# MarToonLi/StableDiffusionEO

Hardware: AMD Instinct MI355X
Metric: 512x512 canny2image images/sec (20 DDIM steps); ms per UNet step reported alongside (higher is better)
Workload: dtype f16; 1 GPU; SD1.5 + ControlNet-canny 512x512, batch=1 per GPU (CFG pair fused, N=2), 20 DDIM steps + VAE decode, fp16 storage / fp32 accumulate (BASELINE configs[1]); model_config=sd15, ddim_steps=20, parallelism=dp1 (image index -> rank, RCCL all_gather of final latents), weights=seeded synthetic (no checkpoint in the container)

## Files before the change

### stablediffusioneo_amd/csrc/api_ops.hip

```cpp
#include <stdarg.h>

#include "../../include/sdeo.h"
#include "sdeo_internal.h"
#include "kernels.h"

namespace sdeo {

static thread_local std::string g_last_error;

void set_error(const std::string& msg) { g_last_error = msg; }

int fail(const char* fmt, ...) {
  char buf[1024];
  va_list ap;
  va_start(ap, fmt);
  vsnprintf(buf, sizeof(buf), fmt, ap);
  va_end(ap);
  g_last_error = buf;
  return 1;
}

}

using namespace sdeo;
// ... 296 lines not shown
                              int ldres, int m, int n, int k, float* stats, int stats_ld, int* strips_out, void* stream) {
  const Fp8Arm arm = disarm_fp8();
  SDEO_CHECK(stats && strips_out, "gemm_stats: null argument");
  ConvGemm p;
  fill_gemm(p, m, n, k);
  p.x = (const f16*)x; p.w = (const f16*)w; p.bias = bias; p.res = (const f16*)res; p.y = (f16*)y;
  p.ldx = ldx; p.ldw = ldw; p.ldy = ldy; p.ldres = ldres;
  take_fp8(p, arm);
  *strips_out = conv_gemm_stats_strips(p);
  if (*strips_out == 0) return 0;
  SDEO_CHECK(*strips_out <= stats_ld, "gemm_stats: %d strips do not fit stats_ld %d", *strips_out, stats_ld);
  p.stats_out = stats; p.stats_ld = stats_ld;
  return conv_gemm(p, S(stream));
}

int sdeo_debug_gemm_res_rows_f16(void* y, int ldy, const void* x, int ldx, const void* w, int ldw, const float* bias, const void* res,
                                 int ldres, int res_rows, int m, int n, int k, float* stats, int stats_ld, int* strips_out, void* workspace,
                                 size_t workspace_bytes, void* stream) {
  const Fp8Arm arm = disarm_fp8();
  ConvGemm p;
  fill_gemm(p, m, n, k);
  p.x = (const f16*)x; p.w = (const f16*)w; p.bias = bias; p.res = (const f16*)res; p.y = (f16*)y;
  p.ldx = ldx; p.ldw = ldw; p.ldy = ldy; p.ldres = ldres; p.res_rows = res_rows;
  p.workspace = (float*)workspace; p.workspace_bytes = workspace_bytes;
  take_fp8(p, arm);
  if (stats) {
    SDEO_CHECK(strips_out, "gemm_res_rows: null argument");
    *strips_out = conv_gemm_stats_strips(p);
    SDEO_CHECK(*strips_out <= stats_ld, "gemm_res_rows: %d strips do not fit stats_ld %d", *strips_out, stats_ld);
    if (*strips_out > 0) { p.stats_out = stats; p.stats_ld = stats_ld; }
  }
  return conv_gemm(p, S(stream));
}

int sdeo_debug_conv2d_ex_f16(void* y, const void* x, const void* w_krsc, const float* bias, const void* res, int res_rows, int n, int h,
                             int w, int cin, int cout, int ksize, float* stats, int stats_ld, int* strips_out, const float* ln_stats,
                             const float* ln_s, int ln_ld, int ln_strips, void* workspace, size_t workspace_bytes, void* stream) {
  const Fp8Arm arm = disarm_fp8();
  ConvGemm p;
  if (int rc = fill_conv(p, n, h, w, cin, cout, ksize, 1, 0)) return rc;
  p.x = (const f16*)x; p.w = (const f16*)w_krsc; p.y = (f16*)y; p.bias = bias; p.res = (const f16*)res; p.res_rows = res_rows;
  p.workspace = (float*)workspace; p.workspace_bytes = workspace_bytes;
  take_fp8(p, arm);
  if (ln_stats) { p.ln_stats = ln_stats; p.ln_s = ln_s; p.ln_ld = ln_ld; p.ln_strips = ln_strips; p.ln_c = cin; p.ln_eps = 1e-5f; }
  if (stats) {
    SDEO_CHECK(strips_out, "conv2d_ex: null argument");
    *strips_out = conv_gemm_stats_strips(p);
    SDEO_CHECK(*strips_out > 0 && *strips_out <= stats_ld, "conv2d_ex: %d strips do not fit stats_ld %d", *strips_out, stats_ld);
    p.stats_out = stats; p.stats_ld = stats_ld;
  }
  return conv_gemm(p, S(stream));
}

int sdeo_debug_gemm_multi_f16(int count, const int* tile, const int* splitk, const int* m, const int* n, const int* k, void* const* y,
                              const int* ldy, const void* const* x, const int* ldx, const void* const* w, const int* ldw,
                              const void* const* bias, const void* const* res, const int* ldres, const float* scale, void* stream) {
  (void)disarm_fp8();
  SDEO_CHECK(count >= 1 && tile && splitk && m && n && k && y && ldy && x && ldx && w && ldw && scale, "gemm_multi: null argument");
  std::vector<ConvGemm> ps((size_t)count);
  for (int i = 0; i < count; ++i) {
    ConvGemm& p = ps[i];
    fill_gemm(p, m[i], n[i], k[i]);
    p.x = (const f16*)x[i]; p.w = (const f16*)w[i]; p.y = (f16*)y[i];
    p.bias = bias ? (const float*)bias[i] : nullptr;
    p.res = res ? (const f16*)res[i] : nullptr;
    p.ldx = ldx[i]; p.ldw = ldw[i]; p.ldy = ldy[i]; p.ldres = (res && res[i] && ldres) ? ldres[i] : 0;
    p.scale = scale[i];
    p.force_tile = tile[i]; p.force_splitk = splitk[i];
  }
  ConvGemmMultiPlan pl;
  if (int rc = conv_gemm_multi_plan(ps, tile[0], &pl)) return rc;
  void* tab = nullptr;
  SDEO_HIP(hipMalloc(&tab, pl.table.size()));
  int rc = 0;
  if (hipMemcpy(tab, pl.table.data(), pl.table.size(), hipMemcpyHostToDevice) != hipSuccess) rc = fail("gemm_multi: cannot write the problem table");
  if (!rc) rc = conv_gemm_multi_launch(pl, tab, nullptr, S(stream));
  if (!rc && hipStreamSynchronize(S(stream)) != hipSuccess) rc = fail("gemm_multi: the launch failed");
  (void)hipFree(tab);
  return rc;
}

int sdeo_debug_gemm_ln_f16(void* y, int ldy, const void* x, int ldx, const void* w_folded, int ldw, const float* ln_s,
                           const float* bias_folded, const float* stats, int stats_ld, int strips, int ln_c, int m, int n, int k, int act, float eps, void* workspace, size_t workspace_bytes, void* stream) {
  const Fp8Arm arm = disarm_fp8();
  ConvGemm p;
  fill_gemm(p, m, n, k);
  p.x = (const f16*)x; p.w = (const f16*)w_folded; p.bias = bias_folded; p.y = (f16*)y;
  p.ldx = ldx; p.ldw = ldw; p.ldy = ldy; p.act = act;
  p.ln_stats = stats; p.ln_s = ln_s; p.ln_strips = strips; p.ln_ld = stats_ld; p.ln_c = ln_c; p.ln_eps = eps;
  p.workspace = (float*)workspace; p.workspace_bytes = workspace_bytes;
  take_fp8(p, arm);
  return conv_gemm(p, S(stream));
}

int sdeo_debug_row_stats_f16(float* stats, int stats_ld, const void* x, int ldx, int rows, int c, void* stream) {
  return row_stats(stats, stats_ld, (const f16*)x, ldx, rows, c, S(stream));
}

int sdeo_layernorm_f16(void* y, const void* x, const float* gamma, const float* beta, int rows, int c, float eps,
                       void* stream) {
  return layernorm((f16*)y, c, (const f16*)x, c, gamma, beta, rows, c, eps, S(stream));
}

int sdeo_debug_layernorm_ld_f16(void* y, int ldy, const void* x, int ldx, const float* gamma, const float* beta, int rows, int c,
                                float eps, void* stream) {
  SDEO_CHECK(ldx >= c && ldy >= c, "layernorm_ld: ldx=%d ldy=%d below c=%d", ldx, ldy, c);
// ... 117 lines not shown
```

### stablediffusioneo_amd/csrc/conv_gemm.hip

```cpp
#include <stdlib.h>

#include <array>
#include <map>

#include <type_traits>
#include <utility>

#include "conv_inl.h"

namespace sdeo {

template <int BM, int BN, int STAGES, bool UPS, bool WS, bool W8 = false, int KPB = 1, bool MX = false, bool MULTI = false, int EPI = EPI_STAGED>
__global__ __launch_bounds__(WS ? 512 : 256) void conv_gemm_dma_kernel(const std::conditional_t<MULTI, MPArgs, KP> pp) {
  kernarg_warm<sizeof(pp)>();
  static_assert(!MULTI || (!W8 && !MX), "multi-problem launches stream fp16 weights");
  static_assert(EPI == EPI_STAGED || (!W8 && !MX && !MULTI && !UPS), "the register-direct epilogue exists for the plain fp16 kernels");
  KP pl;
  int wg = blockIdx.x;
  [[maybe_unused]] int mp_prob = 0;
  if constexpr (MULTI) {
    int pre[kMultiMax];
#pragma unroll
    for (int i = 0; i < kMultiMax; ++i) pre[i] = mp_prefix(pp.tab, i);
    int prob = 0, first = 0;
#pragma unroll
    for (int i = 0; i < kMultiMax - 1; ++i) {
      const bool past = (int)blockIdx.x >= pre[i];
      prob += past ? 1 : 0;
      first = past ? pre[i] : first;
    }
    mp_prob = __builtin_amdgcn_readfirstlane(min(prob, pp.count - 1));
    wg = __builtin_amdgcn_readfirstlane((int)blockIdx.x - first);
    pl = mp_block(pp.tab, mp_prob);
    pl.scale = pp.scale[mp_prob];
    mp_globalize(pl);
  } else {
    pl = pp;
  }
  asm volatile("" : "+s"(pl.M), "+s"(pl.N), "+s"(pl.K), "+s"(pl.Hi), "+s"(pl.Wi), "+s"(pl.Cin), "+s"(pl.Wo),
               "+s"(pl.S), "+s"(pl.stride), "+s"(pl.pad), "+s"(pl.HoWo), "+s"(pl.ldx), "+s"(pl.ldw), "+s"(pl.nk),
               "+s"(pl.nk_per_split), "+s"(pl.tiles_m), "+s"(pl.tiles_n), "+s"(pl.n_fastest));
  const KP& p = pl;
  static_assert(!MX || (WS && !W8 && !UPS && KPB == 1), "the block-scaled fp8 path exists for the plain wave-specialised GEMM");
  constexpr int BK = 64, RPP = 32;
  constexpr int WRPP = W8 ? 64 : 32;
  constexpr int XP = BM / RPP, WP = (BN + WRPP - 1) / WRPP, L = XP + WP;
  constexpr int TM = BM / 2, TN = BN / 2, MI = TM / 16, NI = TN / 16;
  constexpr int XBYTES = BM * BK * 2, WBYTES = WP * 4096, STAGE = XBYTES + WBYTES;
  constexpr int PF = STAGES - KPB;
  constexpr int FLY = STAGES - 2 * KPB;
  static_assert(KPB >= 1 && FLY >= 0 && PF >= 1 && STAGES <= 10, "ring depth");

  extern __shared__ __attribute__((aligned(16))) char smem[];

  const int wave_all = __builtin_amdgcn_readfirstlane(threadIdx.x >> 6);
  const bool do_load = !WS || wave_all >= 4;
  const bool do_mma = !WS || wave_all < 4;
  const int tid = threadIdx.x & 255, lane = tid & 63, wave = tid >> 6;
  const int wm = wave & 1, wn = wave >> 1;
  int m0, n0;
  auto set_tile = [&](int t) {
    const int tile = xcd_remap(t, p.tiles_m * p.tiles_n);
    const int tm = p.n_fastest ? tile / p.tiles_n : tile % p.tiles_m;
    const int tn = p.n_fastest ? tile % p.tiles_n : tile / p.tiles_m;
    m0 = tm * BM; n0 = tn * BN;
  };
  set_tile(wg);
  const int z = blockIdx.z;
// ... 92 lines not shown
      }
    }
#pragma unroll
    for (int i = 0; i < WP; ++i) {
      __builtin_amdgcn_global_load_lds((const __attribute__((address_space(1))) void*)wptr[i],
                                       (__attribute__((address_space(3))) void*)(wsm + i * 4096), 16, 0, 0);
      wptr[i] += winc[i];
    }
    if (++st_c == tapsteps) {
      st_c = 0;
      if (++st_s == p.S) { st_s = 0; ++st_r; }
    }
  };
  auto retire = [&](int g) {
    const int ahead = max(0, min(FLY, nk - (g + 1) * KPB));
    static_for<FLY + 1>([&](auto A) {
      if (ahead == A.value) wait_vmcnt<A.value * L>();
    });
  };
  auto refill = [&](int g) {
#pragma unroll
    for (int j = 0; j < KPB; ++j) {
      const int step = PF + g * KPB + j;
      if (step < nk && !dbg_on(p, 8)) issue(step % STAGES);
    }
  };
  const int ngroups = (nk + KPB - 1) / KPB;

  if constexpr (WS) {
    if (!do_mma) {
      if (nk > 0) {
#pragma unroll
        for (int s = 0; s < PF; ++s)
          if (s < nk) issue(s);
        for (int g = 0; g < ngroups; ++g) {
          retire(g);
          __builtin_amdgcn_s_barrier();
          refill(g);
        }
      }
      __builtin_amdgcn_s_barrier();
      return;
    }
  }

  const int frow = lane & 15, fq = lane >> 4;
  constexpr int g0 = 0;
  f32x4 acc[NI][MI];
#pragma unroll
  for (int i = 0; i < NI; ++i)
#pragma unroll
    for (int j = 0; j < MI; ++j) acc[i][j] = f32x4{0.f, 0.f, 0.f, 0.f};

  float2* lnsm = reinterpret_cast<float2*>(smem + STAGES * STAGE);
  const bool ln_lds = p.ln_stats != nullptr && p.splitk == 1;
  if (ln_lds && wn == 0) {
    for (int rr = lane; rr < TM; rr += 64) {
      const int m = m0 + wm * TM + rr;
      float r = 0.f, rm = 0.f;
      if (m < p.M) ln_row_scalars(p, m, r, rm);
      lnsm[wm * TM + rr] = make_float2(r, rm);
    }
    asm volatile("s_waitcnt lgkmcnt(0)" ::: "memory");
  }

  f32x4 bpre[NI];
  const bool use_bpre = p.bias && !p.bias_per_row && p.splitk == 1;
#pragma unroll
  for (int i = 0; i < NI; ++i) {
    const int n = n0 + wn * TN + lane_chan<NI, EPI == EPI_DIRECT>(i, fq);
    bpre[i] = (use_bpre && n < p.N) ? *reinterpret_cast<const f32x4*>(p.bias + n) : f32x4{0.f, 0.f, 0.f, 0.f};
  }

  constexpr bool DB = (NI + MI) * 8 + NI * MI * 4 <= 200;
  const unsigned lds0 = (unsigned)(size_t)(__attribute__((address_space(3))) char*)smem;
  const int swl = (frow >> 1) & 7;
  const unsigned xa0 = lds0 + (wm * TM + frow) * 128 + ((fq ^ swl) << 4), xa1 = lds0 + (wm * TM + frow) * 128 + (((4 + fq) ^ swl) << 4);
  const int g8 = (fq + 2 * ((frow >> 2) & 3)) & 7;
  const unsigned wa0 = W8 ? lds0 + XBYTES + (wn * TN + frow) * 64 + g8 * 8 : xa0 + XBYTES + (wn * TN - wm * TM) * 128;
  const unsigned wa1 = W8 ? lds0 + XBYTES + (wn * TN + frow) * 64 + (g8 ^ 4) * 8 : xa1 + XBYTES + (wn * TN - wm * TM) * 128;
  constexpr int WSTEP = W8 ? 1024 : 2048;
  typedef std::conditional_t<W8, uint2, f16x8> wfrag;
  auto widen = [](const wfrag& w) -> f16x8 {
    if constexpr (W8) {
      const f16x2 a = __builtin_amdgcn_cvt_scalef32_pk_f16_fp8(w.x, 1.0f, false), b = __builtin_amdgcn_cvt_scalef32_pk_f16_fp8(w.x, 1.0f, true);
      const f16x2 c = __builtin_amdgcn_cvt_scalef32_pk_f16_fp8(w.y, 1.0f, false), d = __builtin_amdgcn_cvt_scalef32_pk_f16_fp8(w.y, 1.0f, true);
      return f16x8{a[0], a[1], b[0], b[1], c[0], c[1], d[0], d[1]};
    } else {
      return w;
    }
  };
  auto read_half = [&](const char* xs, const char* wsm, int kk, wfrag (&wf)[NI], f16x8 (&xf)[MI]) {
#pragma unroll
    for (int i = 0; i < NI; ++i) {
      const int row = wn * TN + i * 16 + frow;
      if constexpr (W8) wf[i] = *reinterpret_cast<const uint2*>(wsm + row * 64 + ((kk * 4 + fq + 2 * ((row >> 2) & 3)) & 7) * 8);
      else wf[i] = *reinterpret_cast<const f16x8*>(wsm + row * 128 + swz_chunk<64>(row, kk * 4 + fq) * 16);
    }
#pragma unroll
    for (int j = 0; j < MI; ++j) {
      const int row = wm * TM + j * 16 + frow;
      xf[j] = *reinterpret_cast<const f16x8*>(xs + row * 128 + swz_chunk<64>(row, kk * 4 + fq) * 16);
    }
  };
  auto mma_half = [&](const wfrag (&wf)[NI], const f16x8 (&xf)[MI]) {
#pragma unroll
    for (int i = 0; i < NI; ++i) {
      const f16x8 w = widen(wf[i]);
#pragma unroll
      for (int j = 0; j < MI; ++j)
        acc[i][j] = __builtin_amdgcn_mfma_f32_16x16x32_f16(w, xf[j], acc[i][j], 0, 0, 0);
    }
  };
  auto compute = [&](int it) {
    if constexpr (DB) {
      const unsigned sb = ((g0 + it) % STAGES) * STAGE;
      wfrag wf0[NI], wf1[NI];
      f16x8 xf0[MI], xf1[MI];
      static_for<NI>([&](auto I) { lds_read_w<I.value * WSTEP>(wf0[I.value], wa0 + sb); });
      static_for<MI>([&](auto J) { lds_read128<J.value * 2048>(xf0[J.value], xa0 + sb); });
      static_for<NI>([&](auto I) { lds_read_w<I.value * WSTEP>(wf1[I.value], wa1 + sb); });
      static_for<MI>([&](auto J) { lds_read128<J.value * 2048>(xf1[J.value], xa1 + sb); });
      asm volatile("s_waitcnt lgkmcnt(%0)" ::"n"(NI + MI) : "memory");
      __builtin_amdgcn_sched_barrier(0);
      mma_half(wf0, xf0);
      __builtin_amdgcn_sched_barrier(0);
      asm volatile("s_waitcnt lgkmcnt(0)" ::: "memory");
// ... 20 lines not shown
      __builtin_amdgcn_s_waitcnt(0xc07f);
      if constexpr (MX) {
        typedef int v8i __attribute__((ext_vector_type(8)));
        typedef int v4i __attribute__((ext_vector_type(4)));
        const unsigned xm0 = lds0 + (wm * TM + frow) * 128 + ((fq ^ swl) << 4), xm1 = lds0 + (wm * TM + frow) * 128 + (((4 + fq) ^ swl) << 4);
        const unsigned wm0 = xm0 + XBYTES + (wn * TN - wm * TM) * 128, wm1 = xm1 + XBYTES + (wn * TN - wm * TM) * 128;
        f16x8 wlo[NI], whi[NI], xlo[MI], xhi[MI];
        int swv[NI], sxv[MI];
        const unsigned char* swp[NI];
        const unsigned char* sxp[MI];
#pragma unroll
        for (int i = 0; i < NI; ++i) {
          const int n = n0 + wn * TN + i * 16 + frow;
          swp[i] = p.mx_sw + (size_t)(n < p.N ? n : 0) * p.mx_ldsw + kbeg * 4 + fq;
        }
#pragma unroll
        for (int j = 0; j < MI; ++j) {
          const int m = m0 + wm * TM + j * 16 + frow;
          sxp[j] = p.mx_sx + (size_t)(m < p.M ? m : 0) * p.mx_ldsx + kbeg * 4 + fq;
        }
        auto rd = [&](unsigned sb) {
          static_for<NI>([&](auto I) { lds_read128<I.value * 2048>(wlo[I.value], wm0 + sb); lds_read128<I.value * 2048>(whi[I.value], wm1 + sb); });
          static_for<MI>([&](auto J) { lds_read128<J.value * 2048>(xlo[J.value], xm0 + sb); lds_read128<J.value * 2048>(xhi[J.value], xm1 + sb); });
        };
        auto cat = [](const f16x8& lo, const f16x8& hi) -> v8i {
          const v4i a = __builtin_bit_cast(v4i, lo), b = __builtin_bit_cast(v4i, hi);
          return v8i{a[0], a[1], a[2], a[3], b[0], b[1], b[2], b[3]};
        };
        __builtin_amdgcn_s_barrier();
        rd(0u);
        for (int it = 0; it < nk; ++it) {
          int swn[NI], sxn[MI];
#pragma unroll
          for (int i = 0; i < NI; ++i) swv[i] = swp[i][it * 4];
#pragma unroll
          for (int j = 0; j < MI; ++j) sxv[j] = sxp[j][it * 4];
          (void)swn; (void)sxn;
          asm volatile("s_waitcnt lgkmcnt(0)" ::: "memory");
          __builtin_amdgcn_sched_barrier(0);
#pragma unroll
          for (int i = 0; i < NI; ++i) {
            const v8i w = cat(wlo[i], whi[i]);
#pragma unroll
            for (int j = 0; j < MI; ++j)
              acc[i][j] = __builtin_amdgcn_mfma_scale_f32_16x16x128_f8f6f4(w, cat(xlo[j], xhi[j]), acc[i][j], 0, 0, 0, swv[i], 0, sxv[j]);
          }
          __builtin_amdgcn_sched_barrier(0);
          if (it + 1 < nk) {
            __builtin_amdgcn_s_barrier();
            rd(((it + 1) % STAGES) * STAGE);
          }
        }
      } else if constexpr (DB) {
        wfrag wf0[NI], wf1[NI];
        f16x8 xf0[MI], xf1[MI];
        auto reads0 = [&](unsigned sb) {
          if (dbg_on(p, 16)) return;
          static_for<NI>([&](auto I) { lds_read_w<I.value * WSTEP>(wf0[I.value], wa0 + sb); });
          static_for<MI>([&](auto J) { lds_read128<J.value * 2048>(xf0[J.value], xa0 + sb); });
        };
        auto reads1 = [&](unsigned sb) {
          if (dbg_on(p, 16)) return;
          static_for<NI>([&](auto I) { lds_read_w<I.value * WSTEP>(wf1[I.value], wa1 + sb); });
          static_for<MI>([&](auto J) { lds_read128<J.value * 2048>(xf1[J.value], xa1 + sb); });
        };
        stamp(p, 1);
        __builtin_amdgcn_s_barrier();
        stamp(p, 2);
        reads0((g0 % STAGES) * STAGE);
        reads1((g0 % STAGES) * STAGE);
        int ing = 1;
        for (int it = 0; it < nk; ++it) {
          const bool more = it + 1 < nk;
          if (ing == KPB) ing = 0;
          const bool newgroup = KPB == 1 || ing == 0;
          const unsigned sbn = ((g0 + it + 1) % STAGES) * STAGE;
          asm volatile("s_waitcnt lgkmcnt(%0)" ::"n"(NI + MI) : "memory");
          __builtin_amdgcn_sched_barrier(0);
          if (!dbg_on(p, 4)) mma_half(wf0, xf0);
          __builtin_amdgcn_sched_barrier(0);
          if (newgroup || !more) {
            asm volatile("s_waitcnt lgkmcnt(0)" ::: "memory");
            __builtin_amdgcn_sched_barrier(0);
            if (more) {
              __builtin_amdgcn_s_barrier();
              reads0(sbn);
            }
          } else {
            reads0(sbn);
            asm volatile("s_waitcnt lgkmcnt(%0)" ::"n"(NI + MI) : "memory");
          }
          __builtin_amdgcn_sched_barrier(0);
          if (!dbg_on(p, 4)) mma_half(wf1, xf1);
          __builtin_amdgcn_sched_barrier(0);
          if (more) reads1(sbn);
          ++ing;
        }
      } else {
        for (int it = 0; it < nk; ++it) {
          if (it % KPB == 0) __builtin_amdgcn_s_barrier();
          if (!dbg_on(p, 4)) compute(it);
        }
      }
    } else {
#pragma unroll
      for (int s = 0; s < PF; ++s)
        if (s < nk) issue(s);
      for (int it = 0; it < nk; ++it) {
        if (it % KPB == 0) {
          retire(it / KPB);
          __builtin_amdgcn_s_barrier();
          refill(it / KPB);
        }
        compute(it);
      }
    }
  }
  KP pe = p;
  if constexpr (MULTI) { pe = mp_block(pp.tab, mp_prob); pe.scale = pp.scale[mp_prob]; }
  pin_epilogue_scalars(pe);
  __builtin_amdgcn_s_barrier();
  stamp(p, 3);
  if (dbg_on(p, 32)) return;
  static_assert(4 * epilogue_scratch_bytes(TN) <= STAGES * STAGE, "epilogue scratch");
  constexpr int SCR = (STAGES * STAGE / 4) & ~15;
  [[maybe_unused]] constexpr int NBLK = epilogue_blocks(TN, MI, SCR);
  [[maybe_unused]] char* scratch = smem + wave * SCR;
  int mrow[MI];
#pragma unroll
  for (int j = 0; j < MI; ++j) {
    const int m = m0 + wm * TM + j * 16 + frow;
    mrow[j] = m < pe.M ? m : -1;
  }
  const float2* lnrow = ln_lds ? lnsm + wm * TM : nullptr;
  int trip = 0;
#pragma nounroll
  do {
    if constexpr (EPI == EPI_DIRECT) {
      epilogue_direct<NI, MI, TN>(pe, acc, mrow, n0 + wn * TN, fq, bpre, use_bpre, lnrow);
    } else {
      epilogue_rows<NI, MI, TN, NBLK, EPI>(pe, acc, mrow, n0 + wn * TN, fq, z, bpre, use_bpre, scratch, lnrow);
      if (EpiMode<EPI>::gn(pe)) {
        asm volatile("s_waitcnt lgkmcnt(0)" ::: "memory");
        __builtin_amdgcn_s_barrier();
        if (wm == 0) {
          const int bimg = m0 / pe.HoWo;
          gn_partials_finish<TN, 2>(pe, smem + 2 * wn * SCR, SCR, lane, bimg, (m0 - bimg * pe.HoWo) / BM, n0 + wn * TN);
        }
// ... 179 lines not shown
  const float* src = p.ws + (size_t)m * p.N + n;
  const size_t zs = (size_t)p.M * p.N;
  f32x4 bv = f32x4{0.f, 0.f, 0.f, 0.f}, b2 = bv;
  f16x4 rv = f16x4{0, 0, 0, 0};
  if (p.bias) {
    if (p.bias_per_row) bv += p.bias[m];
    else bv = *reinterpret_cast<const f32x4*>(p.bias + n);
  }
  if (p.bias2) b2 = *reinterpret_cast<const f32x4*>(p.bias2 + (size_t)(m / p.HoWo) * p.ld_bias2 + n);
  if (p.res) rv = *reinterpret_cast<const f16x4*>(p.res + (size_t)res_row(p, m) * p.ldres + n);
  for (int z0 = 0; z0 < p.splitk; z0 += 8) {
    f32x4 t[8];
#pragma unroll
    for (int u = 0; u < 8; ++u)
      t[u] = (z0 + u < p.splitk) ? *reinterpret_cast<const f32x4*>(src + (size_t)(z0 + u) * zs) : f32x4{0.f, 0.f, 0.f, 0.f};
#pragma unroll
    for (int u = 0; u < 8; ++u) v += t[u];
  }
  if (p.wscale) v *= *reinterpret_cast<const f32x4*>(p.wscale + n);
  if (p.ln_stats) {
    float r, rm;
    ln_row_scalars(p, m, r, rm);
    v = v * r - *reinterpret_cast<const f32x4*>(p.ln_s + n) * rm;
  }
  v += bv;
  v += b2;
  if (p.act == 1) {
#pragma unroll
    for (int t = 0; t < 4; ++t) v[t] = silu_f(v[t]);
  } else if (p.act == 2) {
#pragma unroll
    for (int t = 0; t < 4; ++t) v[t] = quick_gelu_f(v[t]);
  } else if (p.act == 4) {
#pragma unroll
    for (int t = 0; t < 4; ++t) v[t] = fmaxf(v[t], 0.f);
  } else if (p.act == 5) {
#pragma unroll
    for (int t = 0; t < 4; ++t) v[t] = gelu_erf_f(v[t]);
  }
  v *= p.scale;
#pragma unroll
  for (int t = 0; t < 4; ++t) v[t] += (float)rv[t];
  if (p.y32) {
    *reinterpret_cast<f32x4*>(p.y32 + (size_t)m * p.ldy + n) = v;
  } else {
    f16x4 o;
#pragma unroll
    for (int t = 0; t < 4; ++t) o[t] = (f16)v[t];
    *reinterpret_cast<f16x4*>(p.y + (size_t)m * p.ldy + n) = o;
  }
}

template <typename K>
static int launch_k(K kernel, int smem, DeviceOnce* attr_done, const KP& kp, int tiles, hipStream_t stream, int threads = 256) {
  if (attr_done->need()) {
    SDEO_HIP(hipFuncSetAttribute(reinterpret_cast<const void*>(kernel), hipFuncAttributeMaxDynamicSharedMemorySize, smem));
    attr_done->mark();
  }
  hipLaunchKernelGGL(kernel, dim3(tiles, 1, kp.splitk), dim3(threads), smem, stream, kp);
  SDEO_HIP(hipGetLastError());
  return 0;
}

template <int BM, int BN, int ST, bool UPS, bool WS, bool W8 = false, int KPB = 1, bool MX = false, int EPI = EPI_STAGED>
static int launch_dma(const KP& kp, int tiles, hipStream_t stream) {
  static DeviceOnce done;
  constexpr int smem = ST * (W8 ? BM * 128 + (BN + 63) / 64 * 4096 : (BM + BN) * 128) + BM * 8;
  static_assert(smem <= 160 * 1024, "LDS");
  return launch_k(&conv_gemm_dma_kernel<BM, BN, ST, UPS, WS, W8, KPB, MX, false, EPI>, smem, &done, kp, tiles, stream, WS ? 512 : 256);
}

typedef int (*MultiLaunch)(const MPArgs& a, int tiles, hipStream_t stream);
template <int BM, int BN, int ST, bool WS>
static int launch_dma_multi(const MPArgs& a, int tiles, hipStream_t stream) {
  static DeviceOnce done;
  constexpr int smem = ST * (BM + BN) * 128 + BM * 8;
  static_assert(smem <= 160 * 1024, "LDS");
  auto kernel = &conv_gemm_dma_kernel<BM, BN, ST, false, WS, false, 1, false, true>;
  if (done.need()) {
    SDEO_HIP(hipFuncSetAttribute(reinterpret_cast<const void*>(kernel), hipFuncAttributeMaxDynamicSharedMemorySize, smem));
    done.mark();
  }
  hipLaunchKernelGGL(kernel, dim3(tiles, 1, 1), dim3(WS ? 512 : 256), smem, stream, a);
  SDEO_HIP(hipGetLastError());
  return 0;
}

template <int BM, int BN>
static int launch_generic(const KP& kp, int tiles, hipStream_t stream) {
  static DeviceOnce done;
  return launch_k(&conv_gemm_kernel<BM, BN, 32, true>, 2 * (BM + BN) * 64, &done, kp, tiles, stream);
}

template <int BM, int BN, int ST, int CAPS = 0, int KPB = 1, int KINDS = K_D>
static constexpr TileCfg dma_tile(const char* name) {
  constexpr bool WS = !(CAPS & CAP_LIGHT);
  TileCfg c{BM, BN, 64, ST, TK_DMA, CAPS | (KPB > 1 ? CAP_GROUPED : 0), KPB, 0, 0, name,
            &launch_dma<BM, BN, ST, false, WS, false, KPB>, &launch_dma<BM, BN, ST, true, WS, false, KPB>, nullptr, nullptr, {}};
  c.epi[EPI_STAGED] = c.plain;
  if constexpr ((KINDS & K_D) != 0) c.epi[EPI_DIRECT] = &launch_dma<BM, BN, ST, false, WS, false, KPB, false, EPI_DIRECT>;
  if constexpr ((KINDS & K_SK) != 0) c.epi[EPI_SPLITK] = &launch_dma<BM, BN, ST, false, WS, false, KPB, false, EPI_SPLITK>;
  if constexpr ((KINDS & K_GG) != 0) c.epi[EPI_GEGLU] = &launch_dma<BM, BN, ST, false, WS, false, KPB, false, EPI_GEGLU>;
  if constexpr ((KINDS & K_GN) != 0) c.epi[EPI_GN] = &launch_dma<BM, BN, ST, false, WS, false, KPB, false, EPI_GN>;
  if constexpr ((KINDS & K_GNB) != 0) c.epi[EPI_GN_B2] = &launch_dma<BM, BN, ST, false, WS, false, KPB, false, EPI_GN_B2>;
  if constexpr ((CAPS & CAP_W8) != 0) c.w8 = &launch_dma<BM, BN, ST, false, true, true>;
  if constexpr ((CAPS & CAP_MX) != 0) c.mx = &launch_dma<BM, BN, ST, false, true, false, 1, true>;
  return c;
}
template <int BM, int BN>
static constexpr TileCfg generic_tile(const char* name) {
  return {BM, BN, 32, 2, TK_GENERIC, 0, 1, 0, 0, name, &launch_generic<BM, BN>, &launch_generic<BM, BN>, nullptr, nullptr, {&launch_generic<BM, BN>}};
}
static const TileCfg kTiles[] = {
    dma_tile<128, 128, 3, CAP_MX>("conv_gemm_dma_kernel<128,128,3>"),
    dma_tile<128, 64, 3, CAP_W8 | CAP_MX>("conv_gemm_dma_kernel<128,64,3>"),
    dma_tile<64, 64, 4, CAP_W8, 1, K_D | K_SK | K_GG>("conv_gemm_dma_kernel<64,64,4>"),
    generic_tile<128, 64>("conv_gemm_kernel<128,64,32,true>"),
    generic_tile<64, 64>("conv_gemm_kernel<64,64,32,true>"),
    dma_tile<256, 128, 3>("conv_gemm_dma_kernel<256,128,3>"),
    dma_tile<64, 160, 3, CAP_W8 | CAP_MX, 1, K_D | K_SK | K_GN>("conv_gemm_dma_kernel<64,160,3>"),
    dma_tile<128, 160, 3>("conv_gemm_dma_kernel<128,160,3>"),
    dma_tile<256, 160, 3>("conv_gemm_dma_kernel<256,160,3>"),
    dma_tile<32, 160, 4, CAP_W8>("conv_gemm_dma_kernel<32,160,4>"),
    dma_tile<64, 160, 5>("conv_gemm_dma_kernel<64,160,5>"),
    dma_tile<128, 160, 4>("conv_gemm_dma_kernel<128,160,4>"),
    dma_tile<128, 64, 5>("conv_gemm_dma_kernel<128,64,5>"),
    halo_row(0), halo_row(1), halo_row(2), halo_row(3), halo_row(4), halo_row(5),
    dma_tile<64, 64, 8, CAP_W8>("conv_gemm_dma_kernel<64,64,8>"),
    dma_tile<32, 160, 6, CAP_W8>("conv_gemm_dma_kernel<32,160,6>"),
    dma_tile<128, 128, 4, CAP_MX>("conv_gemm_dma_kernel<128,128,4>"),
    halo_row(6), halo_row(7), halo_row(8), halo_row(9),
    dma_tile<128, 64, 2, CAP_LIGHT, 1, K_D | K_GG>("conv_gemm_dma_kernel<128,64,2>"),
    dma_tile<64, 64, 2, CAP_LIGHT>("conv_gemm_dma_kernel<64,64,2>"),
    dma_tile<128, 128, 2, CAP_LIGHT>("conv_gemm_dma_kernel<128,128,2>"),
    dma_tile<128, 160, 2, CAP_LIGHT, 1, 0>("conv_gemm_dma_kernel<128,160,2>"),
    dma_tile<64, 160, 2, CAP_LIGHT>("conv_gemm_dma_kernel<64,160,2>"),
    dma_tile<32, 160, 2, CAP_LIGHT, 1, 0>("conv_gemm_dma_kernel<32,160,2>"),
    dma_tile<64, 64, 3, CAP_LIGHT>("conv_gemm_dma_kernel<64,64,3>"),
    dma_tile<128, 64, 3, CAP_LIGHT, 1, 0>("conv_gemm_dma_kernel<128,64,3>/4w"),
    halo_row(10), halo_row(11), halo_row(12), halo_row(13), halo_row(14), halo_row(15), halo_row(16),
    dma_tile<32, 160, 6, 0, 2, K_D | K_GN>("conv_gemm_dma_kernel<32,160,6,k2>"),
    dma_tile<64, 64, 8, 0, 2, 0>("conv_gemm_dma_kernel<64,64,8,k2>"),
    dma_tile<64, 64, 9, 0, 3>("conv_gemm_dma_kernel<64,64,9,k3>"),
    dma_tile<64, 160, 5, 0, 2>("conv_gemm_dma_kernel<64,160,5,k2>"),
    dma_tile<128, 64, 6, 0, 2>("conv_gemm_dma_kernel<128,64,6,k2>"),
    dma_tile<64, 64, 6, 0, 2>("conv_gemm_dma_kernel<64,64,6,k2>"),
    dma_tile<128, 128, 4, 0, 2>("conv_gemm_dma_kernel<128,128,4,k2>"),
    dma_tile<32, 160, 5, 0, 2>("conv_gemm_dma_kernel<32,160,5,k2>"),
};
static const int kTileCount = (int)std::size(kTiles);
static bool by_plan_only(const TileCfg& c) { return (c.caps & (CAP_HALO | CAP_LIGHT | CAP_GROUPED)) != 0; }
static const int kNumCU = 256;

struct Plan { int tile; int splitk; int nk; int tiles_m, tiles_n; int epi; };

static bool is_fast(const ConvGemm& p) { return p.Cin % 64 == 0; }
static bool halo_ok(const ConvGemm& p, const TileCfg& c) {
  if (c.kind != TK_HALO) return false;
  return p.R == 3 && p.S == 3 && p.stride == 1 && p.pad == 1 && conv_pad_after(p) == 1 && !p.ups && p.Cin % 64 == 0 && p.act != 3 && !p.bias_per_row &&
         p.Hi % c.ph == 0 && p.Wi % c.pw == 0 && p.Ho == p.Hi && p.Wo == p.Wi;
}
static int plan_tiles_m(const ConvGemm& p, const TileCfg& c) {
  return c.kind == TK_HALO ? p.B * (p.Hi / c.ph) * (p.Wi / c.pw) : cdiv(p.M, c.bm);
}
static int plan_nk(const ConvGemm& p, const TileCfg& c) { return c.kind == TK_HALO ? p.Cin / 64 : cdiv(p.K, c.bk); }

static int g_force_tile = -1, g_force_splitk = 0, g_force_order = -1;
void conv_gemm_debug_force_order(int order) { g_force_order = order; }
void conv_gemm_debug_force(int tile, int splitk) { g_force_tile = tile; g_force_splitk = splitk; }

typedef std::array<int, 10> ShapeKey;
static std::map<ShapeKey, std::pair<int, int>> g_tuned;
static ShapeKey key_of(const ConvGemm& p) {
  return {p.M, p.N, p.K, p.Cin, p.R, p.stride, (p.act == 3 ? 2 : p.ups) + (p.wscale ? 4 : 0) + (p.mx_sx ? 8 : 0), p.Hi, p.Wi, p.B};
}
static bool has_operand_form(const ConvGemm& p, const TileCfg& c) { return (!p.wscale || (c.caps & CAP_W8)) && (!p.mx_sx || (c.caps & CAP_MX)); }

static Plan make_plan(const ConvGemm& p) {
  if (p.plan_B > 0 && p.plan_B != p.B) {
    ConvGemm q = p;
    q.M = p.M / p.B * p.plan_B; q.B = p.plan_B; q.plan_B = 0;
    Plan pl = make_plan(q);
    pl.tiles_m = plan_tiles_m(p, kTiles[pl.tile]);
    return pl;
  }
  Plan best{};
  const bool fast = is_fast(p);
  const int force_tile = p.force_tile >= 0 ? p.force_tile : g_force_tile;
  const int force_sk = p.force_splitk > 0 ? p.force_splitk : g_force_splitk;
  const bool pair = p.act == 3;
  if (force_tile < 0 && force_sk <= 0 && fast) {
    auto it = g_tuned.find(key_of(p));
    if (it != g_tuned.end() && !(pair && ((kTiles[it->second.first].bn / 2) % 32 != 0 || it->second.second != 1))) {
      const TileCfg& c = kTiles[it->second.first];
      if ((c.kind != TK_HALO || halo_ok(p, c)) && has_operand_form(p, c))
        return Plan{it->second.first, it->second.second, plan_nk(p, c), plan_tiles_m(p, c), cdiv(p.N, c.bn)};
    }
  }
  float best_t = 1e30f;
  for (int t = 0; t < kTileCount; ++t) {
    const TileCfg& c = kTiles[t];
// ... 33 lines not shown
      if (tcost < best_t) { best_t = tcost; best = Plan{t, sk, nk, tmn, tnn}; }
    }
  }
  return best;
}

static ConvGemm mx_view(const ConvGemm& p0) {
  ConvGemm p = p0;
  if (p.mx_sx) { p.K /= 2; p.Cin /= 2; p.ldx /= 2; p.ldw /= 2; }
  return p;
}

static int plan_tn(const Plan& pl) { return kTiles[pl.tile].kind == TK_HALO ? kTiles[pl.tile].bn : kTiles[pl.tile].bn / 2; }

int conv_gemm_stats_strips(const ConvGemm& p0) {
  const ConvGemm p = mx_view(p0);
  const Plan pl = make_plan(p);
  return pl.splitk == 1 ? cdiv(p.N, plan_tn(pl)) : 0;
}

bool conv_gemm_plan_is_halo(const ConvGemm& p) { return kTiles[make_plan(mx_view(p)).tile].kind == TK_HALO; }

static int gn_slots_of(const ConvGemm& p, int cpg);
int conv_gemm_gn_slots(const ConvGemm& p0, int cpg) { return gn_slots_of(mx_view(p0), cpg); }
static int gn_slots_of(const ConvGemm& p, int cpg) {
  if (cpg <= 0 || p.N % cpg || p.act == 3 || p.y32 || !p.y || p.bias_per_row || p.stats_out) return 0;
  const Plan pl = make_plan(p);
  const TileCfg& c = kTiles[pl.tile];
  if (pl.splitk != 1 || c.kind == TK_GENERIC || plan_tn(pl) % cpg) return 0;
  if (p.N % 8 || p.ldy % 8 || (reinterpret_cast<uintptr_t>(p.y) & 15) || (p.res && (p.ldres % 8 || (reinterpret_cast<uintptr_t>(p.res) & 15)))) return 0;
  if (c.kind == TK_HALO) return (p.Hi / c.ph) * (p.Wi / c.pw);
  const int hw = p.Ho * p.Wo;
  return hw % c.bm == 0 ? hw / c.bm : 0;
}

size_t conv_gemm_workspace_bytes(const ConvGemm& p0) {
  const ConvGemm p = mx_view(p0);
  const Plan pl = make_plan(p);
  return pl.splitk > 1 ? (size_t)pl.splitk * p.M * p.N * sizeof(float) : 0;
}

const char* conv_gemm_kernel_name(const ConvGemm& p) { return kTiles[make_plan(mx_view(p)).tile].name; }
int conv_gemm_plan_splitk(const ConvGemm& p) { return make_plan(mx_view(p)).splitk; }

void conv_gemm_query_plan(const ConvGemm& p0, int key[10], int* tile, int* splitk) {
  const ConvGemm p = mx_view(p0);
  const ShapeKey k = key_of(p);
  for (int i = 0; i < 10; ++i) key[i] = k[i];
  const Plan pl = make_plan(p);
  *tile = pl.tile;
  *splitk = pl.splitk;
}

static int g_last_tile = -1, g_last_splitk = 0, g_last_epilogue = -1;
void conv_gemm_last_plan(int* tile, int* splitk) { *tile = g_last_tile; *splitk = g_last_splitk; }
int conv_gemm_last_epilogue() { return g_last_epilogue < 0 ? -1 : g_last_epilogue == EPI_DIRECT ? EPI_DIRECT : EPI_STAGED; }
int conv_gemm_last_epilogue_mode() { return g_last_epilogue >= EPI_SPLITK ? g_last_epilogue : 0; }
static int g_force_epi_mode = -1;
void conv_gemm_debug_force_epilogue_mode(int mode) { g_force_epi_mode = mode; }
int conv_gemm_tile_has_epilogue_mode(int tile, int mode) {
  return tile >= 0 && tile < kTileCount && mode >= 0 && mode < EPI_KINDS && mode != EPI_DIRECT && kTiles[tile].epi[mode] != nullptr;
}

static std::map<std::array<int, 5>, int> g_census;
static int census_flags(const KP& kp) {
  return kp.act | (kp.bias2 ? 8 : 0) | (kp.gn_out ? 16 : 0) | (kp.stats_out ? 32 : 0) | (kp.ln_stats ? 64 : 0) | (kp.res ? 128 : 0) | (kp.coalesce ? 256 : 0);
}
int conv_gemm_epilogue_census(int* rows6, int cap, int clear) {
  int n = 0;
  for (auto& kv : g_census) {
    if (n < cap) { for (int i = 0; i < 5; ++i) rows6[n * 6 + i] = kv.first[i]; rows6[n * 6 + 5] = kv.second; }
    ++n;
  }
  if (clear) g_census.clear();
  return n;
}

static int direct_ok(const ConvGemm& p, const KP& kp, const TileCfg& c) {
  static const int on = [] { const char* e = getenv("SDEO_EPI_DIRECT"); return e ? atoi(e) : 1; }();
  return on && c.epi[EPI_DIRECT] && kp.coalesce && p.act != 3 && !p.gn_out && !p.bias2 && !p.ups && !p.wscale && !p.mx_sx;
}
static int staged_mode(const KP& kp) {
  if (kp.wscale || kp.mx_sx || kp.ups) return EPI_STAGED;
  if (kp.splitk > 1) return EPI_SPLITK;
  if (!kp.coalesce || kp.stats_out) return EPI_STAGED;
  if (kp.act == 3) return EPI_GEGLU;
  if (kp.ln_stats || kp.act != 0 || !kp.gn_out) return EPI_STAGED;
  return kp.bias2 ? EPI_GN_B2 : EPI_GN;
}
static int epi_kind(const ConvGemm& p, const KP& kp, const Plan& pl) {
  static const int kinds_on = [] { const char* e = getenv("SDEO_EPI_KINDS"); return e ? atoi(e) : 1; }();
  const TileCfg& c = kTiles[pl.tile];
  if (direct_ok(p, kp, c)) return EPI_DIRECT;
  if (!kinds_on || g_force_epi_mode == 0) return EPI_STAGED;
  const int k = staged_mode(kp);
  return c.epi[k] ? k : EPI_STAGED;
}

static int prepare(const ConvGemm& p, Plan& pl, KP& kp) {
  SDEO_CHECK(p.x && p.w && (p.y || p.y32), "conv_gemm: null operand");
  SDEO_CHECK(p.M > 0 && p.N > 0 && p.K > 0, "conv_gemm: empty problem M=%d N=%d K=%d", p.M, p.N, p.K);
  SDEO_CHECK(p.act >= 0 && p.act <= 5, "conv_gemm: act=%d unsupported (0 none, 1 SiLU, 2 quick-GELU, 3 GEGLU pair, 4 ReLU, 5 erf GELU)", p.act);
  SDEO_CHECK(p.act != 5 || !p.bias2, "conv_gemm: act 5 (erf GELU) is not built with a per-image bias2");
  SDEO_CHECK(p.N % 4 == 0, "conv_gemm: N=%d must be a multiple of 4", p.N);
  SDEO_CHECK(p.Cin % 8 == 0 && p.ldx % 8 == 0 && p.ldw % 8 == 0, "conv_gemm: Cin=%d ldx=%d ldw=%d must be multiples of 8",
             p.Cin, p.ldx, p.ldw);
  SDEO_CHECK(p.K == p.R * p.S * p.Cin, "conv_gemm: K=%d != R*S*Cin=%d", p.K, p.R * p.S * p.Cin);
// ... 36 lines not shown
  kp.ldx = p.ldx; kp.ldw = p.ldw; kp.ldy = p.ldy; kp.ldres = p.ldres; kp.ld_bias2 = p.ld_bias2;
  kp.res_rows = p.res_rows > 0 ? p.res_rows : p.M;
  kp.act = p.act; kp.bias_per_row = p.bias_per_row; kp.scale = p.scale;
  kp.wscale = p.wscale;
  if (p.mx_sx) {
    SDEO_CHECK(p.mx_sw && p.R == 1 && p.S == 1 && p.stride == 1 && !p.ups && !p.wscale && p.Cin % 64 == 0 && !p.bias_per_row,
               "conv_gemm: block-scaled fp8 operands go with a plain GEMM whose K is a multiple of 128");
    SDEO_CHECK(p.mx_ldsx >= p.K / 16 && p.mx_ldsw >= p.K / 16, "conv_gemm: scale rows too short (%d, %d < %d)", p.mx_ldsx, p.mx_ldsw, p.K / 16);
    kp.mx_sx = p.mx_sx; kp.mx_sw = p.mx_sw; kp.mx_ldsx = p.mx_ldsx; kp.mx_ldsw = p.mx_ldsw;
  }
  if (p.ln_stats) {
    SDEO_CHECK(p.ln_s && p.ln_strips >= 1 && p.ln_ld >= p.ln_strips && p.ln_c > 0, "conv_gemm: incomplete LayerNorm-fold arguments");
    SDEO_CHECK(!p.bias_per_row && !p.y32, "conv_gemm: the LayerNorm fold applies to row-major fp16 products only");
    SDEO_CHECK(p.K == p.Cin && p.stride == 1 && !p.ups, "conv_gemm: the LayerNorm fold needs one input row per output row (a %dx%d filter mixes rows with different statistics)", p.R, p.S);
    kp.ln_stats = p.ln_stats; kp.ln_s = p.ln_s; kp.ln_strips = p.ln_strips; kp.ln_ld = p.ln_ld;
    kp.ln_invc = 1.0f / (float)p.ln_c; kp.ln_eps = p.ln_eps;
  }
  if (p.stats_out) {
    const int strips = pl.splitk == 1 ? cdiv(p.N, plan_tn(pl)) : 0;
    SDEO_CHECK(strips >= 1 && p.stats_ld >= strips && p.y && !p.y32 && p.act != 3,
               "conv_gemm: row statistics need an unsplit fp16 plan (strips %d, stats_ld %d)", strips, p.stats_ld);
    kp.stats_out = p.stats_out; kp.stats_ld = p.stats_ld;
  }
  if (p.gn_out) {
    const int slots = gn_slots_of(p, p.gn_cpg);
    SDEO_CHECK(slots > 0 && slots == p.gn_slots && p.gn_groups * p.gn_cpg == p.N,
               "conv_gemm: GroupNorm partials need an unsplit fp16 plan whose strips cover whole groups (slots %d, expected %d)", slots, p.gn_slots);
    kp.gn_out = p.gn_out; kp.gn_cpg = p.gn_cpg; kp.gn_slots = p.gn_slots; kp.gn_groups = p.gn_groups;
  }
  kp.nk = pl.nk; kp.splitk = pl.splitk; kp.nk_per_split = cdiv(pl.nk, pl.splitk);
  kp.tiles_m = pl.tiles_m; kp.tiles_n = pl.tiles_n;
  pl.epi = EPI_STAGED;
  {
    const double xb = (double)p.M * p.Cin * 2.0 * (p.R * p.S > 1 ? 1.3 : 1.0), wb = (double)p.N * p.K * 2.0;
    const double cost_n_fast = xb + 8.0 * wb;
    const double cost_m_fast = (pl.tiles_n < 8 ? pl.tiles_n : 8) * xb + wb * (pl.tiles_n < 8 ? 1.6 : 1.0);
#ifdef SDEO_DEBUG_KERNELS
    { static const int dbg = [] { const char* e = getenv("SDEO_DBG_GEMM"); return e ? atoi(e) : 0; }(); kp.dbg = dbg; }
#endif
    kp.n_fastest = g_force_order >= 0 ? g_force_order : (cost_n_fast < cost_m_fast ? 1 : 0);
    static const int epi = [] { const char* e = getenv("SDEO_EPI_COALESCE"); return e ? atoi(e) : 1; }();
    kp.coalesce = epi && p.y && !p.y32 && pl.splitk == 1 && !p.bias_per_row && p.N % (p.act == 3 ? 16 : 8) == 0 && p.ldy % 8 == 0 &&
                  (reinterpret_cast<uintptr_t>(p.y) & 15) == 0 &&
                  (!p.res || (p.ldres % 8 == 0 && (reinterpret_cast<uintptr_t>(p.res) & 15) == 0));
    SDEO_CHECK(!p.gn_out || kp.coalesce, "conv_gemm: GroupNorm partials need the LDS-transposed epilogue");
  }
  if (pl.splitk > 1) {
    const size_t need = (size_t)pl.splitk * p.M * p.N * sizeof(float);
    SDEO_CHECK(p.workspace && p.workspace_bytes >= need, "conv_gemm: split-K workspace too small (%zu < %zu)",
               p.workspace_bytes, need);
  }
  if (kTiles[pl.tile].kind == TK_HALO) SDEO_CHECK(halo_ok(p, kTiles[pl.tile]), "conv_gemm: halo plan on an ineligible problem");
  pl.epi = epi_kind(p, kp, pl);
  return 0;
}

static int dispatch(const Plan& pl, int ups, bool w8, const KP& kp, hipStream_t stream) {
  if (pl.tile < 0 || pl.tile >= kTileCount) return fail("conv_gemm: bad tile %d", pl.tile);
  const TileCfg& c = kTiles[pl.tile];
  if (pl.epi < 0 || pl.epi >= EPI_KINDS) return fail("conv_gemm: bad epilogue kind %d", pl.epi);
  if (pl.epi != EPI_STAGED && (kp.mx_sx || w8 || ups || !c.epi[pl.epi]))
    return fail("conv_gemm: tile %d has no %s instantiation for this launch", pl.tile, pl.epi == EPI_DIRECT ? "register-direct" : "specialised staged");
  if (pl.epi >= EPI_SPLITK && pl.epi != staged_mode(kp)) return fail("conv_gemm: epilogue kind %d does not match the problem's mode (%d)", pl.epi, staged_mode(kp));
  const TileLaunch launch = pl.epi != EPI_STAGED ? c.epi[pl.epi] : kp.mx_sx ? c.mx : w8 ? c.w8 : ups ? c.ups : c.plain;
  if (!launch) return fail("conv_gemm: tile %d has no %s instantiation", pl.tile, kp.mx_sx ? "block-scaled fp8" : w8 ? "fp8-weight" : "folded-upsample");
  ++g_census[{pl.tile, pl.splitk, kp.mx_sx ? 3 : w8 ? 2 : ups ? 1 : 0, pl.epi, census_flags(kp)}];
  if (int rc = launch(kp, pl.tiles_m * pl.tiles_n, stream)) return rc;
  if (pl.splitk > 1) {
    const int64_t n = (int64_t)kp.M * (kp.N / 4);
    hipLaunchKernelGGL(splitk_reduce_kernel, dim3((unsigned)cdiv64(n, 256)), dim3(256), 0, stream, kp);
    SDEO_HIP(hipGetLastError());
  }
  return 0;
}

int conv_gemm(const ConvGemm& p0, hipStream_t stream) {
  if (p0.mx_sx)
    SDEO_CHECK(p0.K % 128 == 0 && p0.ldx % 16 == 0 && p0.ldw % 16 == 0 && p0.K == p0.Cin, "conv_gemm: block-scaled fp8 GEMM needs K %% 128 == 0 (K=%d, ldx=%d, ldw=%d)", p0.K, p0.ldx, p0.ldw);
  const ConvGemm p = mx_view(p0);
  Plan pl;
  KP kp{};
  if (int rc = prepare(p, pl, kp)) return rc;
  g_last_tile = pl.tile; g_last_splitk = pl.splitk; g_last_epilogue = pl.epi;
  return dispatch(pl, p.ups, p.wscale != nullptr, kp, stream);
}

struct MultiTile { int tile, bm, bn, stages; bool light; MultiLaunch launch; const char* name; };
static const MultiTile kMultiTiles[] = {
    {2, 64, 64, 4, false, &launch_dma_multi<64, 64, 4, true>, "conv_gemm_dma_kernel<64,64,4> multi"},
    {6, 64, 160, 3, false, &launch_dma_multi<64, 160, 3, true>, "conv_gemm_dma_kernel<64,160,3> multi"},
    {26, 128, 64, 2, true, &launch_dma_multi<128, 64, 2, false>, "conv_gemm_dma_kernel<128,64,2> multi"},
};
static const MultiTile* multi_tile(int tile) {
  for (const MultiTile& m : kMultiTiles) {
    const TileCfg& c = kTiles[m.tile];
    if (m.tile == tile && c.kind == TK_DMA && c.bm == m.bm && c.bn == m.bn && c.stages == m.stages && c.kpb == 1 &&
        ((c.caps & CAP_LIGHT) != 0) == m.light)
      return &m;
  }
  return nullptr;
}

int conv_gemm_multi_plan(const std::vector<ConvGemm>& ps, int tile, ConvGemmMultiPlan* out) {
  *out = ConvGemmMultiPlan{};
  SDEO_CHECK(!ps.empty() && (int)ps.size() <= kMultiMax, "conv_gemm_multi: %d problems in one launch (1..%d)", (int)ps.size(), kMultiMax);
  for (const ConvGemm& p : ps) {
    if (tile < 0) tile = p.force_tile;
    SDEO_CHECK(p.force_tile < 0 || p.force_tile == tile, "conv_gemm_multi: mixed tiles (%d and %d): one tile serves all problems of a launch", tile, p.force_tile);
    SDEO_CHECK(p.force_splitk <= 1, "conv_gemm_multi: a split-K plan (factor %d) cannot be part of a multi-problem launch", p.force_splitk);
  }
  const MultiTile* mt = multi_tile(tile);
  SDEO_CHECK(mt, "conv_gemm_multi: tile %d has no multi-problem instantiation", tile);
  MPTable tab{};
  int total = 0;
  for (size_t i = 0; i < ps.size(); ++i) {
    ConvGemm p = ps[i];
    SDEO_CHECK(!p.mx_sx && !p.wscale, "conv_gemm_multi: problem %d: fp16 weights only", (int)i);
    SDEO_CHECK(!p.gn_out && !p.stats_out && !p.ln_stats, "conv_gemm_multi: problem %d: no GroupNorm-partial, row-statistics or LayerNorm-fold epilogue", (int)i);
    SDEO_CHECK(p.act != 3 && !p.ups && p.plan_B == 0, "conv_gemm_multi: problem %d: no GEGLU pair, folded upsample or batch-prefix plan", (int)i);
    SDEO_CHECK(is_fast(p), "conv_gemm_multi: problem %d: Cin=%d must be a multiple of 64", (int)i, p.Cin);
    p.force_tile = tile; p.force_splitk = 1;
    Plan pl;
    if (int rc = prepare(p, pl, tab.kp[i])) return rc;
    SDEO_CHECK(pl.tile == tile && pl.splitk == 1, "conv_gemm_multi: problem %d cannot run unsplit on tile %d", (int)i, tile);
    total += pl.tiles_m * pl.tiles_n;
    tab.prefix[i] = total;
    out->scale[i] = p.scale;
    out->flops += 2.0 * p.M * p.N * (double)p.K;
    out->bytes += 2.0 * ((double)p.M * p.Cin + (double)p.N * p.K + (double)p.M * p.N);
  }
  for (int i = (int)ps.size(); i < kMultiMax; ++i) tab.prefix[i] = 0x7fffffff;
  out->tile = tile; out->count = (int)ps.size(); out->tiles = total; out->name = mt->name;
  out->table.assign(reinterpret_cast<const char*>(&tab), reinterpret_cast<const char*>(&tab) + sizeof(tab));
  return 0;
}

int conv_gemm_multi_launch(const ConvGemmMultiPlan& pl, const void* table_dev, const float* scales, hipStream_t stream) {
// ... 109 lines not shown
```

### stablediffusioneo_amd/csrc/conv_inl.h

```cpp
#pragma once
#include <type_traits>
#include <utility>

#include "kernels.h"

namespace sdeo {

struct KP {
  const f16* x;
  const f16* w;
  f16* y;
  float* y32;
  const float* bias;
  const float* bias2;
  const f16* res;
  float* ws;
  int M, N, K;
  int Hi, Wi, Cin, Ho, Wo, S, stride, pad, ups;
  int HoWo;
  int ldx, ldw, ldy, ldres, ld_bias2;
  int res_rows;
  int act, bias_per_row;
  float scale;
  int nk, nk_per_split, splitk;
  int tiles_m, tiles_n;
  int dbg;
  int n_fastest;
  int coalesce;
  const float* ln_stats;
  const float* ln_s;
  int ln_strips, ln_ld;
  float ln_invc, ln_eps;
  const float* wscale;
  float* stats_out;
  int stats_ld;
  float* gn_out;
  int gn_cpg, gn_slots, gn_groups;
  const unsigned char* mx_sx;
  const unsigned char* mx_sw;
  int mx_ldsx, mx_ldsw;
};

struct MPTable {
  int prefix[kMultiMax];
  KP kp[kMultiMax];
};
struct MPArgs {
  const MPTable* tab;
  int count;
  float scale[kMultiMax];
};
__device__ __forceinline__ int mp_prefix(const MPTable* tab, int i) {
#if defined(__HIP_DEVICE_COMPILE__)
  return ((const __attribute__((address_space(4))) MPTable*)tab)->prefix[i];
#else
  return tab->prefix[i];
#endif
}
__device__ __forceinline__ KP mp_block(const MPTable* tab, int prob) {
#if defined(__HIP_DEVICE_COMPILE__)
  return ((const __attribute__((address_space(4))) MPTable*)tab)->kp[prob];
#else
  return tab->kp[prob];
#endif
}
__device__ __forceinline__ void mp_globalize(KP& q) {
#define SDEO_GLOBAL_PTR(f) q.f = (decltype(q.f))(__attribute__((address_space(1))) std::remove_pointer_t<decltype(q.f)>*)q.f;
  SDEO_GLOBAL_PTR(x) SDEO_GLOBAL_PTR(w) SDEO_GLOBAL_PTR(y) SDEO_GLOBAL_PTR(y32) SDEO_GLOBAL_PTR(bias) SDEO_GLOBAL_PTR(bias2)
  SDEO_GLOBAL_PTR(res) SDEO_GLOBAL_PTR(ws) SDEO_GLOBAL_PTR(ln_stats) SDEO_GLOBAL_PTR(ln_s) SDEO_GLOBAL_PTR(wscale)
  SDEO_GLOBAL_PTR(stats_out) SDEO_GLOBAL_PTR(gn_out) SDEO_GLOBAL_PTR(mx_sx) SDEO_GLOBAL_PTR(mx_sw)
#undef SDEO_GLOBAL_PTR
}

#ifdef SDEO_DEBUG_KERNELS
__device__ __forceinline__ bool dbg_on(const KP& p, int bit) { return (p.dbg & bit) != 0; }
#else
__device__ __forceinline__ constexpr bool dbg_on(const KP&, int) { return false; }
#endif

constexpr int kStampWGs = 4096, kStampSlots = 16;
static __device__ unsigned long long g_stamps[kStampWGs * kStampSlots];
__device__ __forceinline__ void stamp_cycles(const KP& p, int slot) {
  if (dbg_on(p, 64) && threadIdx.x == 0) {
    const int wg = blockIdx.x + gridDim.x * blockIdx.z;
    if (wg < kStampWGs) g_stamps[wg * kStampSlots + slot] = __builtin_amdgcn_s_memtime();
  }
}
__device__ __forceinline__ void stamp(const KP& p, int slot) {
  if (dbg_on(p, 64) && threadIdx.x == 0) {
    const int wg = blockIdx.x + gridDim.x * blockIdx.z;
    if (wg < kStampWGs) g_stamps[wg * kStampSlots + slot] = __builtin_amdgcn_s_memrealtime();
  }
}

// ... 550 lines not shown
                                         const float2* lnrow = nullptr) {
  int mrow[MI];
#pragma unroll
  for (int j = 0; j < MI; ++j) {
    const int m = m0 + wm * TM + j * 16 + frow;
    mrow[j] = m < p.M ? m : -1;
  }
  epilogue_rows<NI, MI, TN, NB>(p, acc, mrow, n0 + wn * TN, fq, z, bpre, use_bpre, scratch, lnrow);
}

template <int TN, int NW>
__device__ __forceinline__ void gn_partials_finish(const KP& p, char* base, int stride, int lane, int b, int slot, int nb) {
  constexpr int GCH = (TN + 63) / 64;
  float2* tot = reinterpret_cast<float2*>(base) + TN;
#pragma unroll
  for (int c = 0; c < GCH; ++c) {
    const int col = c * 64 + lane;
    if (col < TN) {
      float s = 0.f, q = 0.f;
#pragma unroll
      for (int w = 0; w < NW; ++w) { const float2 v = reinterpret_cast<const float2*>(base + w * stride)[col]; s += v.x; q += v.y; }
      tot[col] = make_float2(s, q);
    }
  }
  __builtin_amdgcn_wave_barrier();
  const int cpg = p.gn_cpg;
  const int g = (nb / cpg) + lane;
  if (lane * cpg < TN && nb + lane * cpg < p.N) {
    float s = 0.f, q = 0.f;
    for (int k = 0; k < cpg; ++k) { const float2 v = tot[lane * cpg + k]; s += v.x; q += v.y; }
    reinterpret_cast<float2*>(p.gn_out)[((size_t)b * p.gn_slots + slot) * p.gn_groups + g] = make_float2(s, q);
  }
}

__device__ __forceinline__ int xcd_remap(int wg, int nwg) {
  const int q = nwg >> 3, r = nwg & 7, xcd = wg & 7, idx = wg >> 3;
  return (xcd < r ? xcd * (q + 1) : r * (q + 1) + (xcd - r) * q) + idx;
}

template <int N, typename F, int... Is>
__device__ __forceinline__ void static_for_impl(F&& f, std::integer_sequence<int, Is...>) {
  (f(std::integral_constant<int, Is>{}), ...);
}
template <int N, typename F>
__device__ __forceinline__ void static_for(F&& f) {
  static_for_impl<N>(f, std::make_integer_sequence<int, N>{});
}
template <int OFF>
__device__ __forceinline__ void lds_read128(f16x8& dst, unsigned addr) {
  asm volatile("ds_read_b128 %0, %1 offset:%2" : "=v"(dst) : "v"(addr), "n"(OFF) : "memory");
}

template <int OFF>
__device__ __forceinline__ void lds_read_w(f16x8& dst, unsigned addr) { lds_read128<OFF>(dst, addr); }
template <int OFF>
__device__ __forceinline__ void lds_read_w(uint2& dst, unsigned addr) {
  asm volatile("ds_read_b64 %0, %1 offset:%2" : "=v"(dst) : "v"(addr), "n"(OFF) : "memory");
}

template <int N>
__device__ __forceinline__ void wait_vmcnt() {
  asm volatile("s_waitcnt vmcnt(%0)" ::"n"(N) : "memory");
}


enum TileKind { TK_DMA, TK_GENERIC, TK_HALO };
enum TileCap { CAP_LIGHT = 1, CAP_GROUPED = 2, CAP_W8 = 4, CAP_MX = 8, CAP_HALO = 16 };
typedef int (*TileLaunch)(const KP& kp, int tiles, hipStream_t stream);
struct TileCfg {
  int bm, bn, bk, stages;
  TileKind kind;
  int caps, kpb;
  int ph, pw;
  const char* name;
  TileLaunch plain, ups, w8, mx;
  TileLaunch epi[EPI_KINDS];
};
constexpr int K_D = 1 << EPI_DIRECT, K_SK = 1 << EPI_SPLITK, K_GG = 1 << EPI_GEGLU, K_GN = 1 << EPI_GN, K_GNB = 1 << EPI_GN_B2;
const TileCfg& halo_row(int variant);

}
```

### stablediffusioneo_amd/csrc/kernels.h

```cpp
#pragma once
#include <vector>

#include "common.h"

namespace sdeo {

struct ConvGemm {
  const f16* x = nullptr;
  const f16* w = nullptr;
  f16* y = nullptr;
  float* y32 = nullptr;
  const float* bias = nullptr;
  const float* bias2 = nullptr;
  const f16* res = nullptr;
  float* workspace = nullptr;
  size_t workspace_bytes = 0;
  int M = 0, N = 0, K = 0;
  int B = 1, Hi = 1, Wi = 1, Cin = 0;
  int Ho = 1, Wo = 1, R = 1, S = 1, stride = 1, pad = 0;
  int pad_after = -1;
  int ups = 0;
  int ldx = 0, ldw = 0, ldy = 0, ldres = 0, ld_bias2 = 0;
  int act = 0;
  int bias_per_row = 0;
  float scale = 1.0f;
  int force_tile = -1;
  int force_splitk = 0;
  const float* ln_stats = nullptr;
  const float* ln_s = nullptr;
  int ln_strips = 0, ln_ld = 0;
  int ln_c = 0;
  float ln_eps = 1e-5f;
  const float* wscale = nullptr;
  float* stats_out = nullptr;
  int stats_ld = 0;
  float* gn_out = nullptr;
  int gn_cpg = 0, gn_slots = 0, gn_groups = 0;
  const uint8_t* mx_sx = nullptr;
  const uint8_t* mx_sw = nullptr;
  int mx_ldsx = 0, mx_ldsw = 0;
  int res_rows = 0;
  int plan_B = 0;
};
int conv_gemm(const ConvGemm& p, hipStream_t stream);
inline int conv_pad_after(const ConvGemm& p) { return p.pad_after < 0 ? p.pad : p.pad_after; }
constexpr int kMultiMax = 16;
struct ConvGemmMultiPlan {
  int tile = -1, count = 0, tiles = 0;
  std::vector<char> table;
  float scale[kMultiMax] = {};
  double flops = 0, bytes = 0;
  const char* name = "";
};
int conv_gemm_multi_plan(const std::vector<ConvGemm>& ps, int tile, ConvGemmMultiPlan* out);
int conv_gemm_multi_launch(const ConvGemmMultiPlan& pl, const void* table_dev, const float* scales, hipStream_t stream);
int conv_gemm_gn_slots(const ConvGemm& p, int cpg);
bool conv_gemm_plan_is_halo(const ConvGemm& p);
int conv_gemm_stats_strips(const ConvGemm& p);
int conv_gemm_read_stamps(unsigned long long* out, int n);
int conv_halo_read_stamps(unsigned long long* out, int n);
size_t conv_gemm_workspace_bytes(const ConvGemm& p);
int conv_gemm_plan_splitk(const ConvGemm& p);
void conv_gemm_query_plan(const ConvGemm& p, int key[10], int* tile, int* splitk);
void conv_gemm_last_plan(int* tile, int* splitk);
int conv_gemm_last_epilogue();
int conv_gemm_last_epilogue_mode();
void conv_gemm_debug_force_epilogue_mode(int mode);
int conv_gemm_tile_has_epilogue_mode(int tile, int mode);
int conv_gemm_epilogue_census(int* rows6, int cap, int clear);
int conv_gemm_tile_info(int tile, int* kind, int* bm, int* bn, int* stages, int* caps, const char** name);
const char* conv_gemm_kernel_name(const ConvGemm& p);
void conv_gemm_debug_force(int tile, int splitk);
void conv_gemm_debug_force_order(int order);
int conv_gemm_autotune(const ConvGemm& p, hipStream_t stream);
size_t conv_gemm_autotune_workspace_bytes(const ConvGemm& p);
void conv_gemm_set_tuned(const int key[10], int tile, int splitk);
std::string conv_gemm_tuned_json();

int gn_chunks(int HW);
int groupnorm_nhwc(f16* y, int ldy, const f16* x, int ldx, const float* gamma, const float* beta, int B, int HW, int C,
                   int groups, float eps, int with_silu, float* partials, hipStream_t stream);

struct GnArgs {
  f16* y; const f16* x; const float* gamma; const float* beta; float* partials;
  int ldy, ldx, B, HW, C, groups;
  float eps;
  int with_silu;
  const float* ext_partials = nullptr;
  int ext_nsc = 0;
};
bool groupnorm_is_single_launch(const GnArgs& a);
int gn_fused_threads(const GnArgs& a);
int groupnorm_nhwc(const GnArgs& a, hipStream_t stream);

int layernorm(f16* y, int ldy, const f16* x, int ldx, const float* gamma, const float* beta, int rows, int C, float eps,
              hipStream_t stream);

int attention(f16* o, int ldo, const f16* q, int ldq, const f16* k, int ldk, const f16* v, int ldv, int B, int H,
              int Tq, int Tk, int TkS, int TkSv, int d, float scale, hipStream_t stream, int causal = 0);
struct AttnArgs {
  f16* o; const f16* q; const f16* k; const f16* v;
  int ldo, ldq, ldk, ldv, B, H, Tq, Tk, TkS, TkSv, d;
  float scale;
  int causal;
  int qB = 0;
  int plan_B = 0;
};
int attention(const AttnArgs& a, hipStream_t stream);
const char* attention_kernel_name(int B, int H, int Tq, int Tk, int d, int causal);
struct Attn2Seg {
// ... 73 lines not shown
```

### stablediffusioneo_amd/csrc/net.hip

```cpp
#include "net_handle.h"

namespace {

static int run(Engine* e, const Program& p, hipStream_t s, bool skip_zero_convs = false) {
  if (!skip_zero_convs) return run_program(p, s, &e->prof);
  for (auto& op : p) {
    if (op.zero_conv) continue;
    if (int rc = e->prof.on ? e->prof.record(op, s) : op(s)) return rc;
  }
  return 0;
}

template <typename Tp>
static int dev_alloc(Engine* e, Tp** p, size_t bytes) {
  void* v = nullptr;
  SDEO_HIP(hipMalloc(&v, bytes < 256 ? 256 : bytes));
  e->extra_allocs.push_back(v);
  e->device_bytes += bytes;
  *p = reinterpret_cast<Tp*>(v);
  return 0;
}

static void free_configured(Engine* e) {
  for (void* v : e->extra_allocs) (void)hipFree(v);
  e->extra_allocs.clear();
  for (Lane& l : e->lanes) {
    if (l.base) (void)hipFree(l.base);
    l = Lane();
  }
  for (Program& p : e->prog) p.clear();
  for (auto& px : e->xprog) for (Program& p : px) p.clear();
  for (int j = 0; j < kMaxControlNets - 1; ++j) {
    for (float& v : e->extra_scales[j]) v = 1.0f;
  }
  e->cache.configured_anew();
  e->fp8.mx_launches = 0;
  e->device_bytes = e->ws.slab_bytes + e->fp8.q8_bytes + e->fp8.mx_bytes + e->ws.lora_backup_bytes;
}

static void set_scales(Engine* h, const float* host_scales, int only_mid) {
  const int mid = (int)h->cplan.in.size();
  h->only_mid = only_mid;
  for (int i = 0; i < kMaxControls; ++i) {
    h->scales[i] = host_scales ? host_scales[i] : 1.0f;
    h->eff_scales[0][i] = (only_mid && i != mid) ? 0.0f : h->scales[i];
    for (int j = 1; j <= h->extra; ++j) h->eff_scales[j][i] = (only_mid && i != mid) ? 0.0f : h->extra_scales[j - 1][i];
  }
}

}

extern "C" {

int sdeo_create(const sdeo_config* cfg, sdeo_handle* out) { return sdeo_create_ex(cfg, nullptr, out); }

int sdeo_create_ex(const sdeo_config* cfg, const sdeo_config_ext* ext, sdeo_handle* out) {
  SDEO_CHECK(cfg && out, "sdeo_create: null argument");
  SDEO_CHECK(!ext || ext->size == (int)sizeof(sdeo_config_ext), "sdeo_create_ex: sdeo_config_ext.size is %d, this library's struct has %d bytes",
             ext ? ext->size : 0, (int)sizeof(sdeo_config_ext));
  SDEO_CHECK(cfg->num_levels >= 1 && cfg->num_levels <= 8 && cfg->vae_num_levels >= 1 && cfg->vae_num_levels <= 8,
             "sdeo_create: bad level count");
  SDEO_CHECK(cfg->model_channels % 32 == 0 && cfg->vae_ch % 32 == 0, "sdeo_create: channels must be multiples of 32 (GroupNorm)");
  SDEO_CHECK(cfg->context_dim % 8 == 0, "sdeo_create: context_dim must be a multiple of 8");
  const int nhc = ext && ext->num_head_channels > 0 ? ext->num_head_channels : 0;
  if (!nhc) SDEO_CHECK((cfg->model_channels / cfg->num_heads) % 8 == 0, "sdeo_create: head dim must be a multiple of 8");
  std::unique_ptr<Engine> e(new Engine());
  e->cfg = *cfg;
  e->num_head_channels = nhc;
  e->use_linear = ext && ext->use_linear_in_transformer != 0;
  if (nhc) {
    const UPlan probe = make_uplan(*cfg, true, 0);
    int bad_c = 0;
    for_each_block(probe, [&](const Blk& b) { if (b.kind == B_ATTN && b.cin % nhc != 0 && !bad_c) bad_c = b.cin; });
    SDEO_CHECK(!bad_c, "sdeo_create_ex: num_head_channels %d does not divide the %d channels of an attention block", nhc, bad_c);
    if (!attention_kernel_name(1, 1, 1, 1, nhc, 0)) {
      const std::string why = sdeo_last_error();
      return fail("sdeo_create_ex: num_head_channels %d is not a head dim the attention kernels are built for (%s)", nhc, why.c_str());
    }
  }
  e->uplan = make_uplan(*cfg, true, nhc);
  e->cplan = make_uplan(*cfg, false, nhc);
  SDEO_CHECK(e->cplan.in.size() + 1 <= kMaxControls, "sdeo_create: more than %d control tensors", kMaxControls);
  e->hconvs = hint_convs(*cfg);
  if (const char* at = getenv("SDEO_AUTOTUNE")) e->autotune = atoi(at) != 0;
  if (const char* ov = getenv("SDEO_OVERLAP")) e->overlap = atoi(ov) != 0;
  SDEO_HIP(hipStreamCreateWithFlags(&e->side, hipStreamNonBlocking));
  SDEO_HIP(hipEventCreateWithFlags(&e->ev_fork, hipEventDisableTiming));
  SDEO_HIP(hipEventCreateWithFlags(&e->ev_join, hipEventDisableTiming));
  set_scales(e.get(), nullptr, 0);
// ... 81 lines not shown
    if (int rc = dev_alloc(h, &h->in_hint[j], (size_t)n * c.hint_channels * px * 64 * 4)) return rc;
  if (int rc = dev_alloc(h, &h->in_ctx, (size_t)n * c.context_len * c.context_dim * 4)) return rc;
  if (int rc = dev_alloc(h, &h->in_t, (size_t)n * 8)) return rc;
  if (h->ip_tokens) if (int rc = dev_alloc(h, &h->in_ip, (size_t)n * h->ip_tokens * c.context_dim * 4)) return rc;
  if (int rc = dev_alloc(h, &h->tab_t, (size_t)sdeo_handle_s::kTabRows * 8)) return rc;
  SDEO_HIP(hipMemset(h->tab_t, 0, (size_t)sdeo_handle_s::kTabRows * 8));
  for (int net = 0; net < 2 + h->extra; ++net) {
    if (int rc = dev_alloc(h, &h->emb_all[net], (size_t)n * h->emb_total[net] * 4)) return rc;
    if (int rc = dev_alloc(h, &h->temb_tab[net], (size_t)sdeo_handle_s::kTabRows * h->emb_total[net] * 4)) return rc;
  }
  if (int rc = dev_alloc(h, &h->out_eps, (size_t)n * c.out_channels * px * 4)) return rc;
  if (int rc = dev_alloc(h, &h->vae_in, (size_t)c.vae_z_channels * px * 4)) return rc;
  if (int rc = dev_alloc(h, &h->vae_out, (size_t)c.vae_out_ch * px * 64 * 4)) return rc;
  if (int rc = dev_alloc(h, &h->vae_u8, (size_t)c.vae_out_ch * px * 64)) return rc;
  if (h->vae_encoder) {
    if (int rc = dev_alloc(h, &h->enc_img, (size_t)c.vae_out_ch * px * 64 * 4)) return rc;
    if (int rc = dev_alloc(h, &h->enc_img_u8, (size_t)c.vae_out_ch * px * 64)) return rc;
    if (int rc = dev_alloc(h, &h->enc_noise, (size_t)c.vae_z_channels * px * 4)) return rc;
    if (int rc = dev_alloc(h, &h->enc_z, (size_t)c.vae_z_channels * px * 4)) return rc;
    if (int rc = dev_alloc(h, &h->enc_moments, (size_t)2 * c.vae_z_channels * px * 4)) return rc;
  }
  const int nctrl = (int)h->cplan.in.size() + 1;
  for (int i = 0; i < nctrl; ++i) {
    const int idx = i < (int)h->cplan.in.size() ? i : (int)h->cplan.in.size() - 1;
    const int ds = h->cplan.in_ds[idx];
    const size_t elems = (size_t)n * h->cplan.in_ch[idx] * (latent_h / ds) * (latent_w / ds);
    if (int rc = dev_alloc(h, &h->in_ctrl[i], elems * 4)) return rc;
    if (int rc = dev_alloc(h, &h->out_ctrl[i], elems * 4)) return rc;
  }
  size_t ms = 0, mg = 0, peaks[L_COUNT];
  if (int rc = build_all(h, true, &ms, &mg, peaks)) return rc;
  for (int i = 0; i < L_COUNT; ++i) {
    Lane& l = h->lanes[i];
    l.bytes = peaks[i];
    SDEO_HIP(hipMalloc((void**)&l.base, l.bytes));
    SDEO_HIP(hipMemset(l.base, 0, l.bytes));
    h->device_bytes += l.bytes;
    if (int rc = dev_alloc(h, &l.splitk_ws, l.splitk_ws_bytes = ms)) return rc;
    if (int rc = dev_alloc(h, &l.gn_ws, mg)) return rc;
  }
  if (int rc = build_all(h, false, &ms, &mg, peaks)) return rc;
  SDEO_CHECK(peaks[L_MAIN] == h->lanes[L_MAIN].bytes && peaks[L_SIDE] == h->lanes[L_SIDE].bytes, "sdeo_configure: arena plan not reproducible");
  SDEO_HIP(hipDeviceSynchronize());
  return 0;
}

int sdeo_configure(sdeo_handle h, int n, int latent_h, int latent_w) {
  SDEO_CHECK(h, "sdeo_configure: null handle");
  SDEO_CHECK(n >= 1 && n <= 64, "sdeo_configure: n=%d out of range", n);
  const int maxds = 1 << (h->cfg.num_levels - 1);
  SDEO_CHECK(latent_h >= maxds && latent_w >= maxds && latent_h % maxds == 0 && latent_w % maxds == 0,
             "sdeo_configure: latent %dx%d must be a positive multiple of %d", latent_h, latent_w, maxds);
  SDEO_CHECK(h->fp8.weight_bits != 8 || h->fp8.q8slab, "sdeo_configure: fp8 weights are packed by sdeo_finalize_weights: call it first");
  const int rc = configure_impl(h, n, latent_h, latent_w);
  if (rc) free_configured(h);
  return rc;
}

static int copy_in(void* dst, const void* src, size_t bytes, hipStream_t s) {
  if (dst == src) return 0;
  SDEO_HIP(hipMemcpyAsync(dst, src, bytes, hipMemcpyDeviceToDevice, s));
  return 0;
}

static int stage_inputs(sdeo_handle h, const float* x, const float* hint, const int64_t* t, const float* ctx, int hint_is_new,
                        int ctx_for_net, hipStream_t s) {
  const sdeo_config& c = h->cfg;
  const size_t px = (size_t)h->lh * h->lw;
  if (x) if (int rc = copy_in(h->in_x, x, (size_t)h->N * c.in_channels * px * 4, s)) return rc;
  if (t) if (int rc = copy_in(h->in_t, t, (size_t)h->N * 8, s)) return rc;
  if (hint && hint_is_new) {
    if (int rc = copy_in(h->in_hint[0], hint, (size_t)h->N * c.hint_channels * px * 64 * 4, s)) return rc;
    if (int rc = run(h, h->prog[P_HINT], s)) return rc;
    h->cache.hint_filled(0);
  }
  if (ctx) {
    h->cache.context_staging(ctx_for_net);
    if (int rc = copy_in(h->in_ctx, ctx, (size_t)h->N * c.context_len * c.context_dim * 4, s)) return rc;
    if (ctx_for_net & CacheRecord::UNET) if (int rc = run(h, h->prog[P_CTX_UNET], s)) return rc;
    if (ctx_for_net & CacheRecord::CONTROL)
      for (int j = 0; j <= h->extra; ++j) if (int rc = run(h, cn_prog(h, j, CP_CTX), s)) return rc;
    h->cache.context_filled(ctx_for_net);
  }
  return 0;
}

static int run_x0(sdeo_handle h, hipStream_t s) {
  h->cache.latent_overwritten();
  return run(h, h->prog[P_X0], s);
}

#define REQUIRE_READY(h)                                                                     \
  SDEO_CHECK(h, "null handle");                                                              \
  SDEO_CHECK(h->finalized, "weights not finalized (call sdeo_finalize_weights)");            \
  SDEO_CHECK(configured(h), "not configured (call sdeo_configure)")

static bool has_timestep_row(int flags) { return (flags & SDEO_TIMESTEP_ROW(0)) != 0; }
static int timestep_row(int flags) { return flags >> __builtin_ctz(SDEO_TIMESTEP_ROW(1) ^ SDEO_TIMESTEP_ROW(0)); }

static int select_time(sdeo_handle h, int flags, const int64_t* timesteps, const char* who, int* row_out) {
  const int row = has_timestep_row(flags) ? timestep_row(flags) : -1;
  SDEO_CHECK(row >= 0 || timesteps, "%s: timesteps required", who);
  if (int rc = h->cache.table_row(who, row)) return rc;
  for (int net = 0; net < 2 + h->extra; ++net) {
    h->emb_cur[net] = row >= 0 ? h->temb_tab[net] + (size_t)row * h->emb_total[net] : h->emb_all[net];
    h->emb_ld_cur[net] = row >= 0 ? 0 : h->emb_total[net];
// ... 423 lines not shown
```

### stablediffusioneo_amd/csrc/net_build.hip

```cpp
#include "net_handle.h"

namespace sdeo {

struct RowStats {
  float* p = nullptr;
  int ld = 0, strips = 0, c = 0;
};

struct ConvOpts {
  const float* bias2 = nullptr; int ld_bias2 = 0;
  const float* const* bias2_cur = nullptr; const int* ld_bias2_cur = nullptr; int bias2_off = 0;
  const T* res = nullptr;
  bool res_half = false;
  int act = 0;
  int plan_rows = 0;
  const float* scale_host = nullptr;
  const T* out = nullptr;
  int cout_store = -1;
  RowStats* stats = nullptr;
  const RowStats* ln = nullptr;
  const float* ln_s = nullptr;
  bool gn_next = false;
  const f16* w_ovr = nullptr; const float* b_ovr = nullptr;
  int pad_before = -1, pad_after = -1;
};

struct Builder {
  typedef ConvOpts CO;
  Engine* e;
  const Lane* lane;
  bool dry;
  bool share = false, half = false;
  bool borrowed_plan = false;
  Program* prog = nullptr;
  size_t max_splitk = 0, max_gn = 0;
  std::string err;

  T alloc(int n, int h, int w, int c) {
    T t;
    t.n = n; t.h = h; t.w = w; t.c = c; t.ld = c;
    t.off = lane->arena->alloc((size_t)n * h * w * c * 2);
    t.p = reinterpret_cast<f16*>(lane->base + t.off);
    return t;
  }
  T alloc2d(int rows, int c) { return alloc(1, 1, rows, c); }
  void release(T& t) { t.release(*lane->arena); }
  void advance(T& cur, T next) { release(cur); cur = next; }
  template <class F>
  void on_lane(const Lane* l, F build) { const Lane* saved = lane; lane = l; build(); lane = saved; }
  static bool gn_from_producer() { static const bool on = [] { const char* v = getenv("SDEO_GN_PRODUCER_STATS"); return !v || atoi(v) != 0; }(); return on; }
  void reserve_gn_partials(const ConvGemm& p, T& y) {
    if (!gn_from_producer() || p.N % 32) return;
    const int hw = p.Ho * p.Wo;
    y.gnp_off = lane->arena->alloc((size_t)(p.plan_B ? p.plan_B : p.B) * ((hw + 31) / 32) * 32 * 2 * sizeof(float));
    y.gnp = nullptr;
    y.gn_slots = 0;
  }
  void push(Op op, const char* key = "elementwise", double flops = 0, double bytes = 0, const std::string& tag = std::string()) {
    op.key = key; op.flops = flops; op.bytes = bytes; op.tag = tag;
    if (!dry) prog->push_back(std::move(op));
  }

  const WEntry* W(const std::string& name) {
    const WEntry* w = e->ws.find(name);
    if (!w && err.empty()) err = "unknown weight " + name;
    return w;
  }
  const f16* wptr(const std::string& name) { return W(name) ? e->ws.ptr<f16>(name) : nullptr; }
  const float* vptr(const std::string& name) { return W(name) ? e->ws.ptr<float>(name) : nullptr; }
  const f16* named_w(const std::string& name) { return reinterpret_cast<const f16*>(e->ws.slab + e->named_off.at(name)); }
  const float* named_v(const std::string& name) { return reinterpret_cast<const float*>(e->ws.slab + e->named_off.at(name)); }

  void launch_conv(ConvGemm p, const float* scale_host, RowStats* stats = nullptr, T* gn_y = nullptr, const ConvOpts* lo = nullptr) {
    const int Mplan = p.plan_B && !borrowed_plan ? p.M / p.B * p.plan_B : p.M;
    e->fp8.use_mx(p, Mplan, *this);
    e->fp8.use_fp8_weights(p, Mplan, e->ws.slab);
    const size_t tune_ws = e->autotune ? conv_gemm_autotune_workspace_bytes(p) : 0;
// ... 9 lines not shown
        gn_y->gnp = reinterpret_cast<float*>(lane->base + gn_y->gnp_off);
        gn_y->gn_slots = slots;
        p.gn_out = gn_y->gnp; p.gn_cpg = cpg; p.gn_slots = slots; p.gn_groups = 32;
      }
    }
    if (!dry && !share && getenv("SDEO_DUMP_GEMM"))
      fprintf(stderr, "SDEO_GEMM %d %d %d %d %d %d %d %d %d %d %s\n", p.M, p.N, p.K, p.Cin, p.R, p.stride, p.ups, p.B, p.Hi, p.Wi,
              conv_gemm_kernel_name(p));
    bool stats_by_kernel = false;
    if (stats) {
      stats->c = p.N;
      stats->strips = conv_gemm_stats_strips(p);
      if (stats->strips > 0 && stats->strips <= stats->ld) { p.stats_out = stats->p; p.stats_ld = stats->ld; }
      else { stats->strips = 1; stats_by_kernel = true; }
    }
    const float* const* b2cur = lo ? lo->bias2_cur : nullptr; const int* b2ld = lo ? lo->ld_bias2_cur : nullptr; const int b2off = lo ? lo->bias2_off : 0;
    size_t need = 0;
    Op op = conv_gemm_op(p, lane->splitk(), &need, true, 0, [scale_host, b2cur, b2ld, b2off](ConvGemm& q) {
      if (scale_host) q.scale = *scale_host;
      if (b2cur) { q.bias2 = *b2cur + b2off; q.ld_bias2 = *b2ld; }
    });
    if (!dry) prog->push_back(std::move(op));
    max_splitk = std::max(max_splitk, e->autotune ? tune_ws : need);
    for (auto& t : mx_tmp) release(t);
    mx_tmp.clear();
    if (stats_by_kernel) {
      float* sp = stats->p; const int ld = stats->ld, rows = p.M, C = p.N, ldy = p.ldy; const f16* y = p.y;
      push([=](hipStream_t s) { return row_stats(sp, ld, y, ldy, rows, C, s); }, "row_stats", 0, 2.0 * rows * C,
           "rows" + std::to_string(rows) + " C" + std::to_string(C));
    }
  }

  std::vector<T> mx_tmp;
  RowStats alloc_stats(int rows, int c) {
    RowStats st;
    st.ld = std::max(1, (c + 31) / 32);
    st.c = c;
    T raw = alloc2d(rows, st.ld * 4);
    st.p = reinterpret_cast<float*>(raw.p);
    stats_blocks.push_back(raw);
    return st;
  }
  void release_stats() {
    for (auto& t : stats_blocks) release(t);
    stats_blocks.clear();
  }
  std::vector<T> stats_blocks;

  static void set_ln(ConvGemm& p, const ConvOpts& o) {
    if (!o.ln) return;
    p.ln_stats = o.ln->p; p.ln_s = o.ln_s; p.ln_strips = o.ln->strips; p.ln_ld = o.ln->ld; p.ln_c = o.ln->c; p.ln_eps = 1e-5f;
  }

  T conv(const T& x, const std::string& name, int cout, int k, int stride, int ups, const CO& o = CO()) {
    const WEntry* w = o.w_ovr ? nullptr : W(name + ".weight");
    ConvGemm p;
    const int pad = o.pad_before >= 0 ? o.pad_before : k / 2;
    const int pad_after = o.pad_after >= 0 ? o.pad_after : k / 2;
    const int hv = ups ? 2 * x.h : x.h, wv = ups ? 2 * x.w : x.w;
    const int ho = (hv + pad + pad_after - k) / stride + 1, wo = (wv + pad + pad_after - k) / stride + 1;
    const int cs = o.cout_store > 0 ? o.cout_store : cout;
    T y = o.out ? o.out->view() : alloc(x.n, ho, wo, cs);
    const int n = half ? x.n / 2 : x.n;
    if (w && w->ipad != x.c && err.empty()) err = "conv " + name + ": input has " + std::to_string(x.c) + " channels, weight expects " + std::to_string(w->ipad);
    p.x = x.p; p.y = y.p;
    if (o.w_ovr) { p.w = o.w_ovr; p.bias = o.b_ovr; } else { p.w = wptr(name + ".weight"); p.bias = vptr(name + ".bias"); }
    p.bias2 = o.bias2; p.ld_bias2 = o.ld_bias2;
    if (o.res) { p.res = o.res->p; p.ldres = o.res->ld; }
    p.B = n; p.Hi = x.h; p.Wi = x.w; p.Cin = x.c; p.Ho = ho; p.Wo = wo; p.R = p.S = k; p.stride = stride; p.pad = pad; p.ups = ups;
    if (pad_after != pad) p.pad_after = pad_after;
    p.M = n * ho * wo; p.N = cs; p.K = k * k * x.c;
    if (half) p.plan_B = x.n;
    if (o.res_half) p.res_rows = p.M / 2;
    p.ldx = x.ld; p.ldw = p.K; p.ldy = y.ld; p.act = o.act;
    const bool want_gn = o.gn_next && !o.out && !o.scale_host && cs == y.c;
    if (want_gn) reserve_gn_partials(p, y);
    launch_conv(p, o.scale_host, o.stats, want_gn ? &y : nullptr, &o);
    return y;
  }

  T gemm(const T& x, const f16* w, int ldw, int n, const float* bias, const CO& o = CO(), float* out32 = nullptr, int ld32 = 0) {
    ConvGemm p;
    const int rows = half ? x.rows() / 2 : x.rows();
    T y;
    if (!out32) y = o.out ? o.out->view() : alloc(x.n, x.h, x.w, n);
    p.x = x.p; p.w = w; p.bias = bias;
    if (out32) { p.y32 = out32; p.ldy = ld32; } else { p.y = y.p; p.ldy = y.ld; }
    if (o.res) { p.res = o.res->p; p.ldres = o.res->ld; }
    p.B = rows; p.Cin = x.c; p.M = rows; p.N = n; p.K = x.c;
    p.ldx = x.ld; p.ldw = ldw; p.act = o.act;
    if (half) p.plan_B = x.rows();
    else if (o.plan_rows > rows) { p.plan_B = o.plan_rows; borrowed_plan = true; }
    if (o.res_half) p.res_rows = rows / 2;
    set_ln(p, o);
    if (o.ln && o.ln->c != x.c && err.empty()) err = "LayerNorm statistics of a " + std::to_string(o.ln->c) + "-channel tensor fed to K = " + std::to_string(x.c);
    launch_conv(p, o.scale_host, o.stats);
    borrowed_plan = false;
    return y;
  }

  T gemm_t(const T& x, const f16* w, int ldw, int c, const float* bias_rows) {
    ConvGemm p;
    const int rows = x.rows();
    T y = alloc2d(c, rows);
    p.x = w; p.w = x.p; p.y = y.p; p.bias = bias_rows; p.bias_per_row = bias_rows ? 1 : 0;
    p.B = c; p.Cin = x.c; p.M = c; p.N = rows; p.K = x.c;
    p.ldx = ldw; p.ldw = x.ld; p.ldy = rows;
    launch_conv(p, nullptr);
    return y;
  }

  T gn(const T& x, const std::string& name, float eps, int silu_, const T* out = nullptr) {
    T y = out ? out->view() : alloc(x.n, x.h, x.w, x.c);
    const float* g = vptr(name + ".weight");
    const float* b = vptr(name + ".bias");
    const int B = half ? x.n / 2 : x.n, HW = x.h * x.w, C = x.c;
    max_gn = std::max(max_gn, (size_t)B * gn_chunks(HW) * 32 * 2 * sizeof(float));
    const Lane* ws = lane;
    const f16* xp = x.p; f16* yp = y.p; const int ldx = x.ld, ldy = y.ld;
    GnArgs ga{yp, xp, g, b, nullptr, ldy, ldx, B, HW, C, 32, eps, silu_};
    const bool apply_only = x.gnp && !groupnorm_is_single_launch(ga);
    if (apply_only) {
      ga.ext_partials = x.gnp; ga.ext_nsc = x.gn_slots;
      max_gn = std::max(max_gn, (size_t)B * 32 * 2 * sizeof(float));
    }
    push([=](hipStream_t s) mutable { ga.partials = ws->gn_ws; return groupnorm_nhwc(ga, s); }, "groupnorm", 0,
         (apply_only ? 2.0 : 3.0) * 2.0 * B * HW * C, "C" + std::to_string(C) + " HW" + std::to_string(HW) + (apply_only ? " apply" : ""));
// ... 52 lines not shown
  if (p.mx_sx || weight_bits != 8 || Mplan > 512 || p.Cin % 64 != 0 || p.ups || p.bias_per_row || conv_gemm_plan_is_halo(p)) return;
  auto it = qindex.find((size_t)(reinterpret_cast<const char*>(p.w) - slab));
  if (it == qindex.end()) return;
  const QRegion& q = qregions[it->second];
  if (q.cols != p.ldw || p.N > q.rows) return;
  p.w = reinterpret_cast<const f16*>(q8slab + q.q_off);
  p.wscale = reinterpret_cast<const float*>(q8slab + q.s_off);
}

}

namespace {

static T build_resblock(Builder& b, const std::string& p, bool vae, const T& x, int cin, int cout, Builder::CO o1, const T* out = nullptr) {
  static const char* const nm[2][5] = {{".in_layers.0", ".in_layers.2", ".out_layers.0", ".out_layers.3", ".skip_connection"},
                                       {".norm1", ".conv1", ".norm2", ".conv2", ".nin_shortcut"}};
  const float eps = vae ? 1e-6f : 1e-5f;
  o1.gn_next = true;
  T h1 = b.gn_conv(x, p + nm[vae][0], eps, 1, p + nm[vae][1], cout, o1);
  T skip;
  if (cin != cout) skip = b.conv(x, p + nm[vae][4], cout, 1, 1, 0);
  Builder::CO o2;
  o2.res = cin != cout ? &skip : &x;
  o2.out = out;
  o2.gn_next = true;
  T y = b.gn_conv(h1, p + nm[vae][2], eps, 1, p + nm[vae][3], cout, o2);
  b.release(h1);
  if (cin != cout) b.release(skip);
  return y;
}
static T build_vae_res(Builder& b, const std::string& p, const T& x, int cin, int cout) { return build_resblock(b, p, true, x, cin, cout, Builder::CO()); }

static T build_res(Builder& b, const std::string& ns, const Blk& blk, const T& x, int net, const T* out = nullptr) {
  const std::string p = ns + blk.name;
  b.half = b.share;
  Builder::CO o1;
  o1.bias2_off = b.e->emb_row.at(p);
  o1.bias2 = b.e->emb_all[net] + o1.bias2_off;
  o1.ld_bias2 = b.e->emb_total[net];
  o1.bias2_cur = &b.e->emb_cur[net];
  o1.ld_bias2_cur = &b.e->emb_ld_cur[net];
  T y = build_resblock(b, p, false, x, blk.cin, blk.cout, o1, out);
  b.half = false;
  return y;
}

static T build_attn(Builder& b, const std::string& ns, const Blk& blk, const T& x, const T& kv, const T* kv_ip, const T* out = nullptr) {
  const sdeo_config& c = b.e->cfg;
  const std::string p = ns + blk.name;
  const std::string t = p + ".transformer_blocks.0";
  const int C = blk.cin, H = blk.heads, d = C / H, N = x.n, Tq = x.h * x.w;
  const int TkS = round8(c.context_len);
  b.half = b.share;
  T g = b.gn(x, p + ".norm", 1e-6f, 0);
  RowStats st0 = b.alloc_stats(x.rows(), C), st1 = b.alloc_stats(x.rows(), C), st2 = b.alloc_stats(x.rows(), C);
  Builder::CO pi; pi.stats = &st0;
  T tok = b.conv(g, p + ".proj_in", C, 1, 1, 0, pi);
  b.release(g);
  Builder::CO l1; l1.ln = &st0; l1.ln_s = b.named_v(t + ".attn1.qkv_ln.s");
  T qkv = b.gemm(tok, b.named_w(t + ".attn1.qkv_ln.w"), C, 3 * C, b.named_v(t + ".attn1.qkv_ln.b"), l1);
  T o1 = b.alloc(x.n, x.h, x.w, C);
  b.attn(o1, qkv.p, 3 * C, qkv.p + C, 3 * C, qkv.p + 2 * C, 3 * C, N, H, Tq, Tq, Tq, Tq, d);
  b.release(qkv);
  Builder::CO r1; r1.res = &tok; r1.stats = &st1;
  T tok1 = b.gemm(o1, b.wptr(t + ".attn1.to_out.0.weight"), C, C, b.vptr(t + ".attn1.to_out.0.bias"), r1);
  b.release(o1);
  b.release(tok);
  Builder::CO l2; l2.ln = &st1; l2.ln_s = b.named_v(t + ".attn2.q_ln.s");
  T q2 = b.gemm(tok1, b.named_w(t + ".attn2.q_ln.w"), C, C, b.named_v(t + ".attn2.q_ln.b"), l2);
  b.half = false;
  T o2 = b.alloc(x.n, x.h, x.w, C);
  if (kv_ip) b.attn(o2, q2.p, C, kv.p, 2 * C, kv.p + C, 2 * C, N, H, Tq, c.context_len, TkS, TkS, d, b.share ? N / 2 : 0,
                    kv_ip->p, kv_ip->p + C, 2 * C, b.e->ip_tokens, round8(b.e->ip_tokens));
  else b.attn(o2, q2.p, C, kv.p, 2 * C, kv.p + C, 2 * C, N, H, Tq, c.context_len, TkS, TkS, d, b.share ? N / 2 : 0);
  b.release(q2);
  T cat = b.alloc(x.n, x.h, x.w, 5 * C);
  const T gg = cat.view(0, 4 * C), tok2v = cat.view(4 * C, C);
  Builder::CO r2; r2.res = &tok1; r2.res_half = b.share; r2.stats = &st2; r2.out = &tok2v;
  T tok2 = b.gemm(o2, b.wptr(t + ".attn2.to_out.0.weight"), C, C, b.vptr(t + ".attn2.to_out.0.bias"), r2);
  b.release(o2);
  b.release(tok1);
  {
    Builder::CO og; og.act = 3; og.out = &gg; og.ln = &st2; og.ln_s = b.named_v(t + ".ff1_ln.s");
    b.gemm(tok2, b.named_w(t + ".ff1_ln.w"), C, 8 * C, b.named_v(t + ".ff1_ln.b"), og);
  }
  b.release_stats();
  Builder::CO ro; ro.res = &x; ro.res_half = b.share; ro.out = out; ro.gn_next = true;
  ro.w_ovr = b.named_w(t + ".ffproj.w"); ro.b_ovr = b.named_v(t + ".ffproj.b");
  T y = b.conv(cat, p + ".proj_out", C, 1, 1, 0, ro);
  b.release(cat);
  return y;
}

static void build_time_embed(Builder& b, const std::string& ns, int net, int rows, const int64_t* tp, float* out) {
  const sdeo_config& c = b.e->cfg;
  const int mc = c.model_channels, emb = 4 * mc, total = b.e->emb_total[net];
  T te = b.alloc2d(rows, mc);
  {
    f16* o = te.p;
    b.push([=](hipStream_t s) { return timestep_embedding(o, tp, rows, mc, s); });
  }
  Builder::CO a; a.act = 1; a.plan_rows = Engine::kTabRows;
  Builder::CO last; last.plan_rows = Engine::kTabRows;
  b.advance(te, b.gemm(te, b.wptr(ns + "time_embed.0.weight"), mc, emb, b.vptr(ns + "time_embed.0.bias"), a));
  b.advance(te, b.gemm(te, b.wptr(ns + "time_embed.2.weight"), emb, emb, b.vptr(ns + "time_embed.2.bias"), a));
  b.gemm(te, b.named_w(ns + "emb_all.weight"), emb, total, b.named_v(ns + "emb_all.bias"), last, out, total);
  b.release(te);
}

static std::vector<const Blk*> attn_blocks(const UPlan& p) {
  std::vector<const Blk*> v;
// ... 482 lines not shown
```

### stablediffusioneo_amd/csrc/net_handle.h

```cpp
#pragma once
#include <cmath>
#include <functional>
#include <memory>
#include <unordered_map>
#include <vector>

#include "../../include/sdeo.h"
#include "cache_record.h"
#include "handle_common.h"
#include "net_plan.h"

namespace sdeo {

static inline int round8(int c) { return (c + 7) / 8 * 8; }

struct FoldJob { size_t w_out, s_out, b_out, w_in; std::string gamma, beta, bias; int rows, C; };
struct ComposeJob { size_t w_out, b_out; std::string wp, bp, w2, b2; int C; };
struct QRegion { size_t off; int rows, cols; size_t q_off, s_off; };

struct Builder;

struct Fp8State {
  std::vector<QRegion> qregions;
  std::unordered_map<size_t, int> qindex;
// ... 37 lines not shown
using namespace sdeo;

struct sdeo_handle_s {
  sdeo_config cfg;
  int num_head_channels = 0;
  bool use_linear = false;
  UPlan uplan, cplan;
  std::vector<HintConv> hconvs;
  WeightStore ws;
  std::unordered_map<std::string, size_t> named_off;
  std::vector<FoldJob> folds;
  std::vector<ComposeJob> composes;
  Fp8State fp8;
  bool finalized = false;
  int emb_total[kNets] = {0};
  std::unordered_map<std::string, int> emb_row;
  int N = 0, lh = 0, lw = 0;
  Lane lanes[L_COUNT];
  hipStream_t side = nullptr;
  hipEvent_t ev_fork = nullptr, ev_join = nullptr;
  bool overlap = true;
  float* in_x = nullptr; float* in_hint[kMaxControlNets] = {nullptr}; float* in_ctx = nullptr; int64_t* in_t = nullptr;
  float* in_ctrl[kMaxControls] = {nullptr};
  float* out_eps = nullptr;
  float* out_ctrl[kMaxControls] = {nullptr};
  float* vae_in = nullptr; float* vae_out = nullptr; uint8_t* vae_u8 = nullptr;
  bool vae_encoder = false;
  float* enc_img = nullptr; uint8_t* enc_img_u8 = nullptr; float* enc_noise = nullptr; float* enc_z = nullptr; float* enc_moments = nullptr;
  int enc_from_u8 = 0, enc_with_noise = 0;
  int ip_tokens = 0;
  float* in_ip = nullptr;
  float ip_scale = 1.0f;
  std::vector<void*> extra_allocs;
  T ctrl[kMaxControls];
  T cn_h[kMaxControlNets][kMaxControls];
  float scales[kMaxControls];
  float eff_scales[kMaxControlNets][kMaxControls];
  int only_mid = 0;
  int extra = 0;
  Program xprog[kMaxControlNets - 1][CP_COUNT];
  float extra_scales[kMaxControlNets - 1][kMaxControls];
  CacheRecord cache;
  static constexpr int kTabRows = SDEO_MAX_TABLE_STEPS;
  float* emb_all[kNets] = {nullptr};
  float* temb_tab[kNets] = {nullptr};
  int64_t* tab_t = nullptr;
  const float* emb_cur[kNets] = {nullptr};
  int emb_ld_cur[kNets] = {0};
  T x0;
  T eps16;
  Program prog[P_COUNT];
  std::vector<size_t> ctrl_elems;
  size_t device_bytes = 0;
  bool autotune = false;
  Profiler prof;
};

static_assert(kMaxControlNets == CacheRecord::kMaxNets, "the cache record keeps one hint entry per control network");

namespace sdeo {

typedef sdeo_handle_s Engine;

static const char* conv_suffix(BlkKind k) { return k == B_DOWN ? ".op" : k == B_UP ? ".conv" : ""; }

static std::string net_ns(int net) { return net == 0 ? NS_UNET : net == 1 ? NS_CN : "control_model_" + std::to_string(net - 1) + "."; }

static Program& cn_prog(Engine* e, int j, CnProg k) {
  static const ProgId kCnProg0[CP_COUNT] = {P_HINT, P_CTX_CN, P_CN, P_CN_SH, P_TEMB_CN};
  return j == 0 ? e->prog[kCnProg0[k]] : e->xprog[j - 1][k];
}

static bool configured(const Engine* e) { return e->lanes[L_MAIN].base != nullptr; }

static inline hipStream_t S(void* s) { return reinterpret_cast<hipStream_t>(s); }

void build_registry(Engine* e);
void reg_extra_controlnets(Engine* e, int count);
void reg_vae_encoder(Engine* e);
void reg_ip_adapter(Engine* e);
int build_all(Engine* e, bool dry, size_t* max_splitk, size_t* max_gn, size_t peaks[L_COUNT]);

}
```

### stablediffusioneo_amd/csrc/net_weights.hip

```cpp
#include "net_handle.h"

namespace {

struct Registry {
  Engine* e;
  bool quant = true;
  void region(size_t off, int rows, int cols) {
    if (!quant) return;
    e->fp8.qindex[off] = (int)e->fp8.qregions.size();
    e->fp8.qregions.push_back(QRegion{off, rows, cols, 0, 0});
  }
  size_t take(size_t bytes) { return e->ws.take(bytes); }
  void add(const std::string& name, WKind kind, std::initializer_list<int64_t> dims, size_t off, int ipad = 0) {
    e->ws.add(name, kind, dims, off, ipad);
  }
  void conv(const std::string& name, int cin, int cout, int k, int opad = -1) {
    const int ip = round8(cin);
    const int op = opad < 0 ? cout : opad;
    const size_t off = take((size_t)op * k * k * ip * 2);
    add(name + ".weight", W_CONV, {cout, cin, k, k}, off, ip);
    region(off, op, k * k * ip);
    add(name + ".bias", W_VEC, {cout}, take((size_t)op * 4));
  }
  void lin(const std::string& name, int cin, int cout, bool bias) {
// ... 250 lines not shown
        q.s_off = align_up(sz, 256); sz = q.s_off + (size_t)q.rows * 4;
      }
      h->fp8.q8_bytes = align_up(sz, 256);
      SDEO_HIP(hipMalloc((void**)&h->fp8.q8slab, h->fp8.q8_bytes));
      h->device_bytes += h->fp8.q8_bytes;
    }
    for (const QRegion& q : h->fp8.qregions)
      if (int rc = quantize_fp8_rows(reinterpret_cast<uint8_t*>(h->fp8.q8slab + q.q_off), reinterpret_cast<float*>(h->fp8.q8slab + q.s_off),
                                     reinterpret_cast<f16*>(h->ws.slab + q.off), q.rows, q.cols, q.cols, q.cols, 0))
        return rc;
    for (const FoldJob& f : h->folds)
      if (int rc = row_sums_f16(reinterpret_cast<float*>(h->ws.slab + f.s_out), reinterpret_cast<const f16*>(h->ws.slab + f.w_out), f.rows, f.C, 0))
        return rc;
  }
  for (const ComposeJob& cj : h->composes) {
    if (int rc = compose_proj(reinterpret_cast<f16*>(h->ws.slab + cj.w_out), reinterpret_cast<float*>(h->ws.slab + cj.b_out),
                              h->ws.ptr<f16>(cj.wp), h->ws.ptr<float>(cj.bp), h->ws.ptr<f16>(cj.w2), h->ws.ptr<float>(cj.b2), cj.C, 4 * cj.C, 0))
      return rc;
  }
  if (h->fp8.act_bits == 8) {
    if (!h->fp8.mxslab) {
      size_t sz = 0;
      for (const QRegion& q : h->fp8.qregions) {
        if (q.cols % 128) continue;
        Fp8State::MxRegion m{};
        m.rows = q.rows; m.cols = q.cols;
        m.q_off = align_up(sz, 256); sz = m.q_off + (size_t)q.rows * q.cols;
        m.s_off = align_up(sz, 256); sz = m.s_off + (size_t)q.rows * (q.cols / 32);
        h->fp8.mxindex[q.off] = m;
      }
      h->fp8.mx_bytes = align_up(sz, 256);
      SDEO_HIP(hipMalloc((void**)&h->fp8.mxslab, h->fp8.mx_bytes < 256 ? 256 : h->fp8.mx_bytes));
      h->device_bytes += h->fp8.mx_bytes;
    }
    for (auto& kv : h->fp8.mxindex)
      if (int rc = quantize_mx(reinterpret_cast<uint8_t*>(h->fp8.mxslab + kv.second.q_off), reinterpret_cast<uint8_t*>(h->fp8.mxslab + kv.second.s_off),
                               reinterpret_cast<const f16*>(h->ws.slab + kv.first), kv.second.rows, kv.second.cols, kv.second.cols, kv.second.cols,
                               kv.second.cols / 32, 0))
        return rc;
  }
  SDEO_HIP(hipDeviceSynchronize());
  return 0;
}

int sdeo_set_activation_precision(sdeo_handle h, int bits, int min_rows) {
  SDEO_CHECK(h, "sdeo_set_activation_precision: null handle");
  SDEO_CHECK(bits == 16 || bits == 8, "sdeo_set_activation_precision: %d bits unsupported (16 or 8)", bits);
  SDEO_CHECK(!h->finalized && !configured(h), "sdeo_set_activation_precision: call it before sdeo_finalize_weights / sdeo_configure");
  h->fp8.act_bits = bits;
  h->fp8.mx_min_rows = min_rows > 0 ? min_rows : 2048;
  return 0;
}
int sdeo_debug_mx_launches(sdeo_handle h) { return h ? h->fp8.mx_launches : -1; }

int sdeo_set_weight_precision(sdeo_handle h, int bits) {
  SDEO_CHECK(h, "sdeo_set_weight_precision: null handle");
  SDEO_CHECK(bits == 16 || bits == 8, "sdeo_set_weight_precision: %d bits unsupported (16 or 8)", bits);
  SDEO_CHECK(!h->finalized && !configured(h), "sdeo_set_weight_precision: call it before sdeo_finalize_weights / sdeo_configure");
  h->fp8.weight_bits = bits;
  return 0;
}

int sdeo_lora_apply(sdeo_handle h, const char* name, const float* down, const float* up, int rank, float scale, void* stream) {
  SDEO_CHECK(h, "sdeo_lora_apply: null handle");
  SDEO_CHECK(!is_ip_weight(name), "sdeo_lora_apply: %s belongs to the image-prompt adapter: adapters on the ip matrices are not supported "
             "(the cached image-prompt K / V rely on them never changing)", name);
  const char* not_ready = !h->finalized ? "weights not finalized (call sdeo_finalize_weights)"
                          : h->fp8.weight_bits == 8 ? "this handle holds fp8 weights (sdeo_set_weight_precision 8): its fp16 copies are the dequantised values, "
                                                      "not the raw ones, and adapters on it are not supported"
                                                    : nullptr;
  const size_t before = h->ws.lora_backup_bytes;
  const int rc = h->ws.lora_apply("sdeo_lora_apply", name, name ? name : "", down, up, rank, scale, not_ready, S(stream));
  h->device_bytes += h->ws.lora_backup_bytes - before;
  return rc;
}

int sdeo_lora_commit(sdeo_handle h) {
  SDEO_CHECK(h, "sdeo_lora_commit: null handle");
  SDEO_CHECK(h->finalized, "sdeo_lora_commit: weights not finalized (call sdeo_finalize_weights)");
  h->ws.lora_release_stage();
  if (int rc = derive_weights(h)) return rc;
  h->cache.weights_changed();
  return 0;
}

int sdeo_lora_clear(sdeo_handle h) {
  SDEO_CHECK(h, "sdeo_lora_clear: null handle");
  SDEO_CHECK(h->finalized, "sdeo_lora_clear: weights not finalized (call sdeo_finalize_weights)");
  const size_t before = h->ws.lora_backup_bytes;
  const int rc = h->ws.lora_restore();
  h->device_bytes -= before - h->ws.lora_backup_bytes;
  if (rc) return rc;
  return sdeo_lora_commit(h);
}

int sdeo_lora_touched(sdeo_handle h) { return h ? h->ws.lora_touched() : 0; }

int sdeo_read_weight(sdeo_handle h, const char* name, float* out) {
  SDEO_CHECK(h, "sdeo_read_weight: null handle");
  return h->ws.read("sdeo_read_weight", name, name ? name : "", out);
}

}
```

### stablediffusioneo_amd/csrc/norm.hip

```cpp
#include <stdlib.h>

#include "kernels.h"

namespace sdeo {

struct GnOne {
  f16* y; const f16* x; const float* gamma; const float* beta; float* partials; int ldy, ldx;
};
struct GnPair { GnOne k[1]; };

int gn_chunks(int HW) { const int c = cdiv(HW, 8); return c > 128 ? 128 : (c < 1 ? 1 : c); }

static int gn_vec_per_block(int C, int groups) {
  const int nvec = C / 8, cpg = C / groups;
  for (int parts = 1; parts <= nvec; ++parts) {
    if (nvec % parts) continue;
    const int nvb = nvec / parts;
    if (nvb > 256) continue;
    if ((nvb * 8) % cpg) continue;
    return nvb;
  }
  return 0;
}

__global__ __launch_bounds__(256) void gn_stats_kernel(const GnPair gp, int Bper, int HW, int C, int cpg, int nvb, int nchunks,
                                                       int groups, int ppc) {
  kernarg_warm<sizeof(GnPair) + 24>();
  const GnOne& g1 = gp.k[0];
  const f16* __restrict__ x = g1.x;
  const int ldx = g1.ldx;
  float* __restrict__ partials = g1.partials;
  __shared__ float s_sum[256 * 8];
  __shared__ float s_sq[256 * 8];
  const int tid = threadIdx.x;
  const int P = 256 / nvb;
  const int cv = tid % nvb, prow = tid / nvb;
  const int chunk = blockIdx.x, part = blockIdx.y, b = blockIdx.z;
  const int c0 = (part * nvb + cv) * 8;
  const int pbeg = chunk * ppc;
  const int pend = min(HW, pbeg + ppc);
  float s[8], q[8];
#pragma unroll
  for (int j = 0; j < 8; ++j) { s[j] = 0.f; q[j] = 0.f; }
  if (prow < P) {
    const f16* base = x + ((size_t)b * HW) * ldx + c0;
    int pix = pbeg + prow;
    for (; pix + 7 * P < pend; pix += 8 * P) {
      f16x8 v[8];
#pragma unroll
      for (int u = 0; u < 8; ++u) v[u] = *reinterpret_cast<const f16x8*>(base + (size_t)(pix + u * P) * ldx);
#pragma unroll
      for (int u = 0; u < 8; ++u)
#pragma unroll
        for (int j = 0; j < 8; ++j) {
// ... 46 lines not shown
    ts += __shfl_xor(ts, off, 64);
    tq += __shfl_xor(tq, off, 64);
  }
  if (gl < gpb && l == 0) {
    const int g = part * gpb + gl;
    float* dst = partials + (((size_t)b * nchunks + chunk) * groups + g) * 2;
    dst[0] = ts;
    dst[1] = tq;
  }
}

__global__ __launch_bounds__(256) void gn_apply_kernel(const GnPair gp, int Bper, int HW, int C, int cpg, int nvb,
                                                       int nchunks, int groups, float eps, int with_silu, int ppc, int nsc) {
  kernarg_warm<sizeof(GnPair) + 24>();
  const GnOne& g1 = gp.k[0];
  f16* __restrict__ y = g1.y;
  const f16* __restrict__ x = g1.x;
  const int ldy = g1.ldy, ldx = g1.ldx;
  const float* __restrict__ gamma = g1.gamma;
  const float* __restrict__ beta = g1.beta;
  const float* __restrict__ partials = g1.partials;
  __shared__ float s_a[256 * 8];
  __shared__ float s_b[256 * 8];
  __shared__ float s_mean[64];
  __shared__ float s_rstd[64];
  const int tid = threadIdx.x;
  const int P = 256 / nvb;
  const int cv = tid % nvb, prow = tid / nvb;
  const int chunk = blockIdx.x, part = blockIdx.y, b = blockIdx.z;
  const int gpb = nvb * 8 / cpg;
  const bool active = prow < P;
  const int c0 = (part * nvb + cv) * 8;
  const int pbeg = chunk * ppc;
  const int pend = min(HW, pbeg + ppc);
  const f16* xb = x + ((size_t)b * HW) * ldx + c0;
  f16* yb = y + ((size_t)b * HW) * ldy + c0;
  f16x8 xv[4];
#pragma unroll
  for (int u = 0; u < 4; ++u) {
    const int pix = pbeg + prow + u * P;
    if (active && pix < pend) xv[u] = *reinterpret_cast<const f16x8*>(xb + (size_t)pix * ldx);
  }
  float gpre[8], bpre[8];
#pragma unroll
  for (int k = 0; k < 8; ++k) {
    const int c = tid + k * 256;
    if (c < nvb * 8) { gpre[k] = gamma[part * nvb * 8 + c]; bpre[k] = beta[part * nvb * 8 + c]; }
  }
  {
    const int tpg = 256 / gpb;
    const int gl = tid / tpg, l = tid - gl * tpg;
    float ts = 0.f, tq = 0.f;
    if (gl < gpb) {
      const float2* src = reinterpret_cast<const float2*>(partials) + ((size_t)b * nsc * groups + part * gpb + gl);
      for (int c0 = l; c0 < nsc; c0 += 8 * tpg) {
        float2 v[8];
#pragma unroll
        for (int u = 0; u < 8; ++u) {
          const int c = c0 + u * tpg;
          v[u] = c < nsc ? src[(size_t)c * groups] : make_float2(0.f, 0.f);
        }
#pragma unroll
        for (int u = 0; u < 8; ++u) { ts += v[u].x; tq += v[u].y; }
      }
    }
    s_a[tid] = ts;
    s_b[tid] = tq;
  }
  __syncthreads();
  if (tid < gpb) {
    const int tpg = 256 / gpb;
    float ts = 0.f, tq = 0.f;
    for (int l = 0; l < tpg; ++l) { ts += s_a[tid * tpg + l]; tq += s_b[tid * tpg + l]; }
    const float inv = 1.0f / ((float)cpg * (float)HW);
    const float mean = ts * inv;
    float var = tq * inv - mean * mean;
    var = var < 0.f ? 0.f : var;
    s_mean[tid] = mean;
    s_rstd[tid] = rsqrtf(var + eps);
  }
  __syncthreads();
#pragma unroll
  for (int k = 0; k < 8; ++k) {
    const int c = tid + k * 256;
    if (c < nvb * 8) {
      const int g = c / cpg;
      const float a = s_rstd[g] * gpre[k];
      s_a[c] = a;
      s_b[c] = bpre[k] - s_mean[g] * a;
    }
  }
  __syncthreads();
  if (!active) return;
  float a[8], bb[8];
#pragma unroll
  for (int j = 0; j < 8; ++j) { a[j] = s_a[cv * 8 + j]; bb[j] = s_b[cv * 8 + j]; }
#pragma unroll
  for (int u = 0; u < 4; ++u) {
    const int pix = pbeg + prow + u * P;
    if (pix < pend) {
      f16x8 o;
#pragma unroll
      for (int j = 0; j < 8; ++j) {
        float f = (float)xv[u][j] * a[j] + bb[j];
        if (with_silu) f = silu_f(f);
        o[j] = (f16)f;
      }
      *reinterpret_cast<f16x8*>(yb + (size_t)pix * ldy) = o;
    }
  }
  for (int pix = pbeg + prow + 4 * P; pix < pend; pix += P) {
    const f16x8 v = *reinterpret_cast<const f16x8*>(xb + (size_t)pix * ldx);
    f16x8 o;
#pragma unroll
    for (int j = 0; j < 8; ++j) {
      float f = (float)v[j] * a[j] + bb[j];
      if (with_silu) f = silu_f(f);
      o[j] = (f16)f;
    }
    *reinterpret_cast<f16x8*>(yb + (size_t)pix * ldy) = o;
  }
}

__global__ __launch_bounds__(256) void gn_fold_partials_kernel(float2* __restrict__ out, const float2* __restrict__ in, int nsc, int groups) {
  __shared__ float2 red[256];
  const int b = blockIdx.x / groups, g = blockIdx.x - b * groups, tid = threadIdx.x;
  float s = 0.f, q = 0.f;
  for (int c = tid; c < nsc; c += 256) { const float2 v = in[((size_t)b * nsc + c) * groups + g]; s += v.x; q += v.y; }
  red[tid] = make_float2(s, q);
  __syncthreads();
  for (int off = 128; off >= 1; off >>= 1) {
    if (tid < off) { red[tid].x += red[tid + off].x; red[tid].y += red[tid + off].y; }
    __syncthreads();
  }
  if (tid == 0) out[(size_t)b * groups + g] = red[0];
}

template <int NT>
__global__ __launch_bounds__(NT) void gn_fused_kernel(const GnPair gp, int Bper, int HW, int cpg, int nvw, int nsweep, float eps,
                                                      int with_silu) {
  kernarg_warm<sizeof(GnPair) + 24>();
  const GnOne& g1 = gp.k[0];
  f16* __restrict__ y = g1.y;
  const f16* __restrict__ x = g1.x;
  const int ldy = g1.ldy, ldx = g1.ldx;
  const float* __restrict__ gamma = g1.gamma;
  const float* __restrict__ beta = g1.beta;
  extern __shared__ __attribute__((aligned(16))) char gsm[];
  const int tid = threadIdx.x, lane = tid & 63, wave = tid >> 6;
  const int wave_u = __builtin_amdgcn_readfirstlane(wave);
  const int P = NT / nvw;
  const int v = tid % nvw, prow = tid / nvw;
  const bool active = prow < P;
  const int part = blockIdx.x, b = blockIdx.y;
  const int c0 = (part * nvw + v) * 8;
  char* slice = gsm;
  float2* part_sq = reinterpret_cast<float2*>(gsm + (size_t)nsweep * NT * 16);
  float2* tot = part_sq + (size_t)2 * nvw * P;
  float* s_mean = reinterpret_cast<float*>(tot + 2 * nvw);
  float* s_rstd = s_mean + 32;

  const f16* xb = x + ((size_t)b * HW) * ldx + c0;
  f16* yb = y + ((size_t)b * HW) * ldy + c0;
  {
    for (int k = 0; k < nsweep; ++k) {
      const int pix = prow + k * P;
      const f16* src = (active && pix < HW) ? xb + (size_t)pix * ldx : x + c0 % 8;
      __builtin_amdgcn_global_load_lds((const __attribute__((address_space(1))) void*)src,
                                       (__attribute__((address_space(3))) void*)(slice + (size_t)k * NT * 16 + wave_u * 1024), 16, 0, 0);
// ... 311 lines not shown
```

### stablediffusioneo_amd/csrc/sdeo_internal.h

```cpp
#ifndef SDEO_INTERNAL_H
#define SDEO_INTERNAL_H

#include <stdint.h>

#ifdef __cplusplus
extern "C" {
#endif

void sdeo_debug_force_gemm_plan(int tile, int splitk);
void sdeo_debug_force_gemm_order(int order);
const char* sdeo_debug_conv2d_kernel_name(int n, int h, int w, int cin, int cout, int ksize, int stride, int upsample2x);
const char* sdeo_debug_attention_kernel_name(int B, int H, int Tq, int Tk, int d, int causal);
const char* sdeo_debug_attention2_kernel_name(int B, int H, int Tq, int Tk, int Tk2, int d);
int sdeo_debug_attention2_check(void* o, int ldo, const void* q, int ldq, const void* k, int ldk, const void* v, int ldv, int tk, int tk_stride,
                                int v_batch_stride, const void* k2, int ldk2, const void* v2, int ldv2, int tk2, int tk2_stride,
                                int v2_batch_stride, float weight2, int b, int heads, int tq, int d, float scale);
int sdeo_debug_conv2d_plan(int n, int h, int w, int cin, int cout, int ksize, int stride, int upsample2x, int act, int fp8, int* key10,
                           int* tile, int* splitk);
int sdeo_debug_gemm_plan(int m, int n, int k, int act, int fp8, int* key10, int* tile, int* splitk);
int sdeo_debug_gemm_multi_f16(int count, const int* tile, const int* splitk, const int* m, const int* n, const int* k, void* const* y,
                              const int* ldy, const void* const* x, const int* ldx, const void* const* w, const int* ldw,
                              const void* const* bias, const void* const* res, const int* ldres, const float* scale, void* stream);
void sdeo_debug_last_gemm_plan(int* tile, int* splitk);
int sdeo_debug_last_gemm_epilogue(void);
int sdeo_debug_last_gemm_epilogue_mode(void);
void sdeo_debug_force_gemm_epilogue_mode(int mode);
int sdeo_debug_tile_has_epilogue_mode(int tile, int mode);
int sdeo_debug_gemm_epilogue_census(int* rows6, int cap, int clear);
int sdeo_debug_tile_info(int tile, int* kind, int* bm, int* bn, int* stages, int* caps, const char** name);
int sdeo_debug_read_stamps(int which, unsigned long long* out, int n);
int sdeo_debug_silu(void* y, const void* x, int64_t n, void* stream);

int sdeo_debug_groupnorm_path(int n, int hw, int c, int groups);
int sdeo_debug_groupnorm_ld_f16(void* y, int ldy, const void* x, int ldx, const float* gamma, const float* beta, int n, int hw, int c,
                                int groups, float eps, int with_silu, void* workspace, void* stream);
int sdeo_debug_layernorm_ld_f16(void* y, int ldy, const void* x, int ldx, const float* gamma, const float* beta, int rows, int c,
                                float eps, void* stream);
int sdeo_debug_softmax_rows(void* p, int ldp, const float* s, int lds, int rows, int cols, float scale, void* stream);

int sdeo_debug_fold_layernorm(void* w_out, float* s_out, float* b_out, const void* w, const float* gamma, const float* beta,
                              const float* bias, int rows, int c, void* stream);
int sdeo_debug_compose_proj(void* w_out, float* b_out, const void* wp, const float* bp, const void* w2, const float* b2, int c, int k2,
                            void* stream);
int sdeo_debug_gemm_stats_f16(void* y, int ldy, const void* x, int ldx, const void* w, int ldw, const float* bias, const void* res,
                              int ldres, int m, int n, int k, float* stats, int stats_ld, int* strips_out, void* stream);
int sdeo_debug_gemm_ln_f16(void* y, int ldy, const void* x, int ldx, const void* w_folded, int ldw, const float* ln_s,
                           const float* bias_folded, const float* stats, int stats_ld, int strips, int ln_c, int m, int n, int k, int act, float eps, void* workspace, size_t workspace_bytes, void* stream);
int sdeo_debug_row_stats_f16(float* stats, int stats_ld, const void* x, int ldx, int rows, int c, void* stream);
int sdeo_debug_conv2d_gn_f16(void* ynorm, void* y, const void* x, const void* w_krsc, const float* bias, const void* res, int n, int h,
                             int w, int cin, int cout, int ksize, int stride, int upsample2x, const float* gamma, const float* beta,
                             int groups, float eps, int with_silu, float* partials, size_t partial_floats, int* slots, void* stream);
int sdeo_debug_conv2d_gn_b2_f16(void* ynorm, void* y, const void* x, const void* w_krsc, const float* bias, const float* bias2, const void* res,
                                int n, int h, int w, int cin, int cout, int ksize, int stride, int upsample2x, const float* gamma,
                                const float* beta, int groups, float eps, int with_silu, float* partials, size_t partial_floats, int* slots,
                                void* stream);

int sdeo_debug_gemm_res_rows_f16(void* y, int ldy, const void* x, int ldx, const void* w, int ldw, const float* bias, const void* res,
                                 int ldres, int res_rows, int m, int n, int k, float* stats, int stats_ld, int* strips_out, void* workspace,
                                 size_t workspace_bytes, void* stream);
int sdeo_debug_conv2d_ex_f16(void* y, const void* x, const void* w_krsc, const float* bias, const void* res, int res_rows, int n, int h,
                             int w, int cin, int cout, int ksize, float* stats, int stats_ld, int* strips_out, const float* ln_stats,
                             const float* ln_s, int ln_ld, int ln_strips, void* workspace, size_t workspace_bytes, void* stream);
int sdeo_debug_attention_qb_f16(void* o, int ldo, const void* q, int ldq, const void* k, int ldk, const void* v, int ldv, int b,
                                int q_batches, int heads, int tq, int tk, int tk_stride, int v_batch_stride, int d, float scale, void* stream);
int sdeo_debug_attention2_qb_f16(void* o, int ldo, const void* q, int ldq, const void* k, int ldk, const void* v, int ldv, int tk,
                                 int tk_stride, int v_batch_stride, const void* k2, int ldk2, const void* v2, int ldv2, int tk2,
                                 int tk2_stride, int v2_batch_stride, float weight2, int b, int q_batches, int heads, int tq, int d,
                                 float scale, void* stream);

int sdeo_debug_quantize_mx(void* q_out, void* scales_out, const void* x, int rows, int cols, void* stream);
int sdeo_debug_gemm_mx_f16(void* y, int ldy, const void* xq, const void* xs, const void* wq, const void* ws, const float* bias, const void* res,
                           int ldres, int m, int n, int k, int act, void* workspace, size_t workspace_bytes, void* stream);
int sdeo_debug_gemm_mx_ex_f16(void* y, int ldy, const void* xq, const void* xs, const void* wq, const void* ws, const float* bias, const void* res,
                              int ldres, int res_rows, int m, int n, int k, int act, float scale, float* stats, int stats_ld, int* strips_out,
                              const float* ln_stats, const float* ln_s, int ln_ld, int ln_strips, int ln_c, float eps, void* workspace,
                              size_t workspace_bytes, void* stream);
int sdeo_debug_quantize_fp8_rows(void* w_f16_inout, void* q_out, float* scale_out, int rows, int cols, void* stream);
void sdeo_debug_next_weights_fp8(const void* q, const float* scale);

int sdeo_debug_mx_launches(sdeo_handle h);

const char* sdeo_debug_fake_scribble_profile(const uint8_t* edges, int h, int w, uint8_t* scribble, float* control_chw, void* workspace,
                                             size_t workspace_bytes, void* stream);

int sdeo_debug_maxpool2x2_f16(void* y, const void* x, int h, int w, int c, void* stream);
const char* sdeo_debug_hed_profile(sdeo_hed_handle h, const uint8_t* img_hwc, void* stream);

#ifdef __cplusplus
}
#endif
#endif
```

### stablediffusioneo_amd/ops.py

```python
from __future__ import annotations

import ctypes as C

import torch

from . import _lib
from ._lib import check, cur_stream, ptr


def _need_cuda(*ts):
    for t in ts:
        if t is not None and not t.is_cuda:
            raise _lib.SdeoError("HIP ops need device tensors (no CPU fallback)")


def _ws(nbytes, device):
    return torch.empty(max(int(nbytes), 16), dtype=torch.uint8, device=device)


def _nhwc_ld(t, what):
    n, h, w, _ = t.shape
    ld = t.stride(2)
    assert t.dtype == torch.float16 and t.stride(3) == 1 and (h == 1 or t.stride(1) == w * ld) and (n == 1 or t.stride(0) == h * w * ld), \
        f"groupnorm: {what} must be fp16 NHWC with unit channel stride and densely stacked pixels (shape {tuple(t.shape)}, strides {t.stride()})"
# ... 129 lines not shown
    check(lib.sdeo_conv2d_nhwc_f16(ptr(y), ptr(x), ptr(w_krsc), ptr(bias), ptr(bias2), ptr(res), *args, act, scale,
                                   ptr(ws), ws.numel(), cur_stream()), "conv2d")
    return y


def conv2d_pad_nhwc(x, w_krsc, pad_before, pad_after, bias=None, bias2=None, res=None, stride=1, upsample2x=False, act=0, scale=1.0):
    lib = _lib.load()
    _need_cuda(x, w_krsc)
    n, h, w, cin = x.shape
    cout, k, _, cin_w = w_krsc.shape
    assert cin == cin_w and x.is_contiguous() and w_krsc.is_contiguous()
    hv, wv = (2 * h, 2 * w) if upsample2x else (h, w)
    ho = (hv + pad_before + pad_after - k) // stride + 1
    wo = (wv + pad_before + pad_after - k) // stride + 1
    y = torch.empty((n, ho, wo, cout), dtype=torch.float16, device=x.device)
    args = (n, h, w, cin, cout, k, stride, int(upsample2x), pad_before, pad_after)
    ws = _ws(lib.sdeo_conv2d_pad_workspace_bytes(*args), x.device)
    check(lib.sdeo_conv2d_pad_nhwc_f16(ptr(y), ptr(x), ptr(w_krsc), ptr(bias), ptr(bias2), ptr(res), *args, act, scale,
                                       ptr(ws), ws.numel(), cur_stream()), "conv2d_pad")
    return y


def conv2d_gn(x, w_krsc, gamma, beta, bias=None, res=None, stride=1, upsample2x=False, groups=32, eps=1e-5, swish=False, bias2=None,
              w8=None, want_partials=False):
    lib = _lib.load()
    _need_cuda(x, w_krsc, gamma, beta)
    n, h, w, cin = x.shape
    cout, k, _, cin_w = w_krsc.shape
    assert cin == cin_w and x.is_contiguous() and w_krsc.is_contiguous()
    hv, wv = (2 * h, 2 * w) if upsample2x else (h, w)
    pad = k // 2
    ho = (hv + 2 * pad - k) // stride + 1
    wo = (wv + 2 * pad - k) // stride + 1
    y = torch.empty((n, ho, wo, cout), dtype=torch.float16, device=x.device)
    yn = torch.empty_like(y)
    pf = n * (ho * wo) * groups * 2 // 16 + n * groups * 2 + 1024
    part = torch.empty(pf, dtype=torch.float32, device=x.device)
    slots = C.c_int(0)
    _arm_fp8(lib, w8)
    if bias2 is None:
        check(lib.sdeo_debug_conv2d_gn_f16(ptr(yn), ptr(y), ptr(x), ptr(w_krsc), ptr(bias), ptr(res), n, h, w, cin, cout, k, stride,
                                           int(upsample2x), ptr(gamma), ptr(beta), groups, eps, int(swish), ptr(part), pf, C.byref(slots),
                                           cur_stream()), "conv2d_gn")
    else:
        assert bias2.shape == (n, cout) and bias2.dtype == torch.float32 and bias2.is_contiguous()
        check(lib.sdeo_debug_conv2d_gn_b2_f16(ptr(yn), ptr(y), ptr(x), ptr(w_krsc), ptr(bias), ptr(bias2), ptr(res), n, h, w, cin, cout, k,
                                              stride, int(upsample2x), ptr(gamma), ptr(beta), groups, eps, int(swish), ptr(part), pf,
                                              C.byref(slots), cur_stream()), "conv2d_gn")
    if slots.value == 0:
        return None
    if want_partials:
        return y, yn, slots.value, part[: n * slots.value * groups * 2].view(n, slots.value, groups, 2)
    return y, yn, slots.value


def conv2d_ex(x, w_krsc, bias=None, res=None, res_rows=0, want_stats=False, ln=None, w8=None):
    lib = _lib.load()
    _need_cuda(x, w_krsc)
    n, h, w, cin = x.shape
    cout, k = w_krsc.shape[0], w_krsc.shape[1]
    assert w_krsc.shape[3] == cin and x.is_contiguous() and w_krsc.is_contiguous()
    y = torch.empty((n, h, w, cout), dtype=torch.float16, device=x.device)
    ld = max(1, (cout + 31) // 32)
    stats = torch.zeros((n * h * w, ld, 2), dtype=torch.float32, device=x.device) if want_stats else None
    strips = C.c_int(0)
    nb = lib.sdeo_conv2d_workspace_bytes(n, h, w, cin, cout, k, 1, 0)
    ws = _ws(nb if w8 is None else max(nb, 64 << 20), x.device)
    lst, lns = ln if ln is not None else (None, None)
    _arm_fp8(lib, w8)
    check(lib.sdeo_debug_conv2d_ex_f16(ptr(y), ptr(x), ptr(w_krsc), ptr(bias), ptr(res), res_rows, n, h, w, cin, cout, k, ptr(stats), ld,
                                       C.byref(strips), ptr(lst), ptr(lns), lst.shape[1] if lst is not None else 0,
                                       1 if lst is not None else 0, ptr(ws), ws.numel(), cur_stream()), "conv2d_ex")
    return y, stats, strips.value


def gemm(x, w, bias=None, res=None, act=0, scale=1.0, out_f32=False, bias_per_row=False, w8=None, out=None):
    lib = _lib.load()
    _need_cuda(x, w)
    m, k = x.shape
    n, k2 = w.shape
    assert k == k2 and x.stride(1) == 1 and w.stride(1) == 1
    y = _out(out, (m, n), torch.float32 if out_f32 else torch.float16, x.device)
    nb = lib.sdeo_gemm_workspace_bytes(m, n, k)
    ws = _ws(nb if w8 is None else max(nb, 64 << 20), x.device)
    _arm_fp8(lib, w8)
    check(lib.sdeo_gemm_f16(ptr(y), n, ptr(x), x.stride(0), ptr(w), w.stride(0), ptr(bias), ptr(res),
                            res.stride(0) if res is not None else 0, m, n, k, act, scale, int(out_f32), int(bias_per_row), ptr(ws),
                            ws.numel(), cur_stream()), "gemm")
    return y


def gemm_multi(problems, tile, tiles=None, splitk=None):
    lib = _lib.load()
    cnt = len(problems)
    outs, keep = [], []
    arr_i = lambda vals: (C.c_int * cnt)(*[int(v) for v in vals])
    arr_p = lambda ts: (C.c_void_p * cnt)(*[t.data_ptr() if t is not None else None for t in ts])
    for p in problems:
        x, w = p["x"], p["w"]
        _need_cuda(x, w)
        assert x.shape[1] == w.shape[1] and x.stride(1) == 1 and w.stride(1) == 1
        y = p.get("out")
        if y is None:
            y = torch.empty((x.shape[0], w.shape[0]), dtype=torch.float16, device=x.device)
        assert y.shape == (x.shape[0], w.shape[0]) and y.stride(1) == 1 and y.dtype == torch.float16
        outs.append(y)
# ... 397 lines not shown
```

Before: 8.708 images/s.

## Fuse input GroupNorm into the proj_in 1x1 conv GEMM mainloop

Adds a GNIN variant of the wave-specialised DMA conv GEMM. It reduces GroupNorm partial sums in the prologue, builds a per-channel scale/shift table in LDS, and applies the affine to the activation fragments before each MFMA. The transformer block's norm followed by proj_in now uses this path when the plan allows, which removes a separate GroupNorm launch and the write and read of the normalised tensor. The cost is extra LDS reads and per-element FMAs inside the inner loop, plus more LDS per block, which can lower occupancy. The shared GN helpers are also factored into a common header.

Result: no change. 8.768 images/s (median of 3 runs) (+0.7%).

```diff
diff --git a/stablediffusioneo_amd/csrc/api_ops.hip b/stablediffusioneo_amd/csrc/api_ops.hip
--- a/stablediffusioneo_amd/csrc/api_ops.hip
+++ b/stablediffusioneo_amd/csrc/api_ops.hip
@@ -372,6 +372,50 @@
   return conv_gemm(p, S(stream));
 }
 
+int sdeo_debug_gn_in_conv2d_f16(void* y, int ldy, const void* x, int ldx, const float* partials, int slots, const float* gamma,
+                                const float* beta, int groups, float eps, const void* w_krsc, const float* bias, int n, int h, int w,
+                                int cin, int cout, int ksize, float* stats, int stats_ld, int* strips_out, int fused, void* xnorm,
+                                void* gn_workspace, const void* xs, const void* ws, void* workspace, size_t workspace_bytes,
+                                int* ran_fused, void* stream) {
+  const Fp8Arm arm = disarm_fp8();
+  if (ran_fused) *ran_fused = 0;
+  SDEO_CHECK(partials && gamma && beta && slots >= 1 && groups >= 1 && cin % groups == 0, "gn_in_conv2d: bad GroupNorm arguments");
+  SDEO_CHECK(ldx >= cin && ldy >= cout, "gn_in_conv2d: ldx=%d ldy=%d below cin=%d cout=%d", ldx, ldy, cin, cout);
+  SDEO_CHECK(fused || (xnorm && gn_workspace && !xs), "gn_in_conv2d: the two-launch form needs xnorm and a GroupNorm workspace");
+  ConvGemm p;
+  if (int rc = fill_conv(p, n, h, w, cin, cout, ksize, 1, 0)) return rc;
+  p.x = (const f16*)x; p.w = (const f16*)w_krsc; p.y = (f16*)y; p.bias = bias; p.ldx = ldx; p.ldy = ldy;
+  p.workspace = (float*)workspace; p.workspace_bytes = workspace_bytes;
+  take_fp8(p, arm);
+  if (xs) { p.mx_sx = (const uint8_t*)xs; p.mx_sw = (const uint8_t*)ws; p.mx_ldsx = p.mx_ldsw = cin / 32; p.ldw = p.K; }
+  if (fused) {
+    p.gn_in = partials; p.gn_in_gamma = gamma; p.gn_in_beta = beta; p.gn_in_slots = slots; p.gn_in_groups = groups; p.gn_in_eps = eps;
+  } else {
+    GnArgs g{(f16*)xnorm, (const f16*)x, gamma, beta, (float*)gn_workspace, cin, ldx, n, h * w, cin, groups, eps, 0};
+    g.ext_partials = partials; g.ext_nsc = slots;
+    if (int rc = groupnorm_nhwc(g, S(stream))) return rc;
+    p.x = (const f16*)xnorm; p.ldx = cin;
+  }
+  if (stats) {
+    SDEO_CHECK(strips_out, "gn_in_conv2d: null argument");
+    *strips_out = conv_gemm_stats_strips(p);
+    SDEO_CHECK(*strips_out > 0 && *strips_out <= stats_ld, "gn_in_conv2d: %d strips do not fit stats_ld %d", *strips_out, stats_ld);
+    p.stats_out = stats; p.stats_ld = stats_ld;
+  }
+  if (int rc = conv_gemm(p, S(stream))) return rc;
+  if (ran_fused) *ran_fused = conv_gemm_last_gn_in();
+  return 0;
+}
+int sdeo_debug_conv2d_plan_has_gn_in(int n, int h, int w, int cin, int cout, int ksize, int groups, int slots) {
+  alignas(256) static float standin[64];
+  ConvGemm p;
+  if (fill_conv(p, n, h, w, cin, cout, ksize, 1, 0)) return 0;
+  if (groups < 1 || cin % groups) return 0;
+  p.x = p.w = (const f16*)standin; p.y = (f16*)standin;
+  p.gn_in = p.gn_in_gamma = p.gn_in_beta = standin; p.gn_in_slots = slots; p.gn_in_groups = groups;
+  return conv_gemm_plan_has_gn_in(p) ? 1 : 0;
+}
+
 int sdeo_debug_gemm_multi_f16(int count, const int* tile, const int* splitk, const int* m, const int* n, const int* k, void* const* y,
                               const int* ldy, const void* const* x, const int* ldx, const void* const* w, const int* ldw,
                               const void* const* bias, const void* const* res, const int* ldres, const float* scale, void* stream) {
diff --git a/stablediffusioneo_amd/csrc/conv_gemm.hip b/stablediffusioneo_amd/csrc/conv_gemm.hip
--- a/stablediffusioneo_amd/csrc/conv_gemm.hip
+++ b/stablediffusioneo_amd/csrc/conv_gemm.hip
@@ -7,13 +7,16 @@
 #include <utility>
 
 #include "conv_inl.h"
+#include "gn_affine.h"
 
 namespace sdeo {
 
-template <int BM, int BN, int STAGES, bool UPS, bool WS, bool W8 = false, int KPB = 1, bool MX = false, bool MULTI = false, int EPI = EPI_STAGED>
+template <int BM, int BN, int STAGES, bool UPS, bool WS, bool W8 = false, int KPB = 1, bool MX = false, bool MULTI = false, int EPI = EPI_STAGED,
+          bool GNIN = false>
 __global__ __launch_bounds__(WS ? 512 : 256) void conv_gemm_dma_kernel(const std::conditional_t<MULTI, MPArgs, KP> pp) {
   kernarg_warm<sizeof(pp)>();
   static_assert(!MULTI || (!W8 && !MX), "multi-problem launches stream fp16 weights");
+  static_assert(!GNIN || (WS && !W8 && !MX && !MULTI && !UPS), "the GroupNorm-of-the-input form exists for the plain wave-specialised fp16 kernels");
   static_assert(EPI == EPI_STAGED || (!W8 && !MX && !MULTI && !UPS), "the register-direct epilogue exists for the plain fp16 kernels");
   KP pl;
   int wg = blockIdx.x;
@@ -212,6 +215,44 @@
 #pragma unroll
     for (int j = 0; j < MI; ++j) acc[i][j] = f32x4{0.f, 0.f, 0.f, 0.f};
 
+  constexpr int GTAB = STAGES * STAGE + BM * 8;
+  if constexpr (GNIN) {
+    constexpr int GT = kGnInMaxC / 4 / 64;
+    float* gtab = reinterpret_cast<float*>(smem + GTAB);
+    const int cpg = p.gn_in_cpg, groups = p.gn_in_groups, tpg = p.gn_in_tpg;
+    const int gw = 64 / tpg;
+    const int g = wave * gw + lane / tpg, l = lane & (tpg - 1);
+    const int cbeg = wave * gw * cpg, cend = min(groups, (wave + 1) * gw) * cpg;
+    float gam[GT], bet[GT];
+#pragma unroll
+    for (int k = 0; k < GT; ++k) {
+      const int c = cbeg + lane + k * 64;
+      gam[k] = 0.f; bet[k] = 0.f;
+      if (c < cend) { gam[k] = p.gn_in_gamma[c]; bet[k] = p.gn_in_beta[c]; }
+    }
+    const int bimg = m0 / p.gn_in_hw;
+    float2 part = make_float2(0.f, 0.f);
+    if (g < groups)
+      part = gn_slot_sum(reinterpret_cast<const float2*>(p.gn_in) + ((size_t)bimg * p.gn_in_slots * groups + g), p.gn_in_slots, groups, l, tpg);
+    float ts = 0.f, tq = 0.f;
+    const int first = lane & ~(tpg - 1);
+    for (int i = 0; i < tpg; ++i) { ts += __shfl(part.x, first + i, 64); tq += __shfl(part.y, first + i, 64); }
+    float mean, rstd;
+    gn_group_stats(ts, tq, cpg, p.gn_in_hw, p.gn_in_eps, mean, rstd);
+#pragma unroll
+    for (int k = 0; k < GT; ++k) {
+      const int c = cbeg + lane + k * 64;
+      const int src = c < cend ? (c / cpg - wave * gw) * tpg : 0;
+      const float gm = __shfl(mean, src, 64), gr = __shfl(rstd, src, 64);
+      if (c < cend) {
+        float a, b;
+        gn_channel_affine(gm, gr, gam[k], bet[k], a, b);
+        gtab[(c >> 3) * 16 + (c & 7)] = a;
+        gtab[(c >> 3) * 16 + 8 + (c & 7)] = b;
+      }
+    }
+  }
+
   float2* lnsm = reinterpret_cast<float2*>(smem + STAGES * STAGE);
   const bool ln_lds = p.ln_stats != nullptr && p.splitk == 1;
   if (ln_lds && wn == 0) {
@@ -233,6 +274,7 @@
   }
 
   constexpr bool DB = (NI + MI) * 8 + NI * MI * 4 <= 200;
+  static_assert(!GNIN || DB, "the GroupNorm-of-the-input form is written into the rotated two-fragment-set loop");
   const unsigned lds0 = (unsigned)(size_t)(__attribute__((address_space(3))) char*)smem;
   const int swl = (frow >> 1) & 7;
   const unsigned xa0 = lds0 + (wm * TM + frow) * 128 + ((fq ^ swl) << 4), xa1 = lds0 + (wm * TM + frow) * 128 + (((4 + fq) ^ swl) << 4);
@@ -359,31 +401,50 @@
           }
         }
       } else if constexpr (DB) {
+        constexpr int TR = GNIN ? 4 : 0, RD = NI + MI + TR;
         wfrag wf0[NI], wf1[NI];
         f16x8 xf0[MI], xf1[MI];
-        auto reads0 = [&](unsigned sb) {
+        [[maybe_unused]] f32x4 gt0[4], gt1[4];
+        [[maybe_unused]] const unsigned ga0 = lds0 + GTAB + fq * 64, ga1 = ga0 + 256;
+        auto reads0 = [&](unsigned sb, [[maybe_unused]] unsigned tb) {
           if (dbg_on(p, 16)) return;
           static_for<NI>([&](auto I) { lds_read_w<I.value * WSTEP>(wf0[I.value], wa0 + sb); });
           static_for<MI>([&](auto J) { lds_read128<J.value * 2048>(xf0[J.value], xa0 + sb); });
+          if constexpr (GNIN) static_for<4>([&](auto Q) { lds_read128<Q.value * 16>(gt0[Q.value], ga0 + tb); });
         };
-        auto reads1 = [&](unsigned sb) {
+        auto reads1 = [&](unsigned sb, [[maybe_unused]] unsigned tb) {
           if (dbg_on(p, 16)) return;
           static_for<NI>([&](auto I) { lds_read_w<I.value * WSTEP>(wf1[I.value], wa1 + sb); });
           static_for<MI>([&](auto J) { lds_read128<J.value * 2048>(xf1[J.value], xa1 + sb); });
+          if constexpr (GNIN) static_for<4>([&](auto Q) { lds_read128<Q.value * 16>(gt1[Q.value], ga1 + tb); });
+        };
+        auto gn_in_apply = [&](f16x8 (&xf)[MI], f32x4 (&gt)[4]) {
+          if constexpr (GNIN) {
+#pragma unroll
+            for (int q = 0; q < 4; ++q) asm volatile("" : "+v"(gt[q]));
+#pragma unroll
+            for (int j = 0; j < MI; ++j) {
+              asm volatile("" : "+v"(xf[j]));
+#pragma unroll
+              for (int e = 0; e < 8; ++e) xf[j][e] = (f16)gn_affine_f32(xf[j][e], gt[e >> 2][e & 3], gt[2 + (e >> 2)][e & 3]);
+            }
+          }
         };
         stamp(p, 1);
         __builtin_amdgcn_s_barrier();
         stamp(p, 2);
-        reads0((g0 % STAGES) * STAGE);
-        reads1((g0 % STAGES) * STAGE);
+        reads0((g0 % STAGES) * STAGE, 0u);
+        reads1((g0 % STAGES) * STAGE, 0u);
         int ing = 1;
         for (int it = 0; it < nk; ++it) {
           const bool more = it + 1 < nk;
           if (ing == KPB) ing = 0;
           const bool newgroup = KPB == 1 || ing == 0;
           const unsigned sbn = ((g0 + it + 1) % STAGES) * STAGE;
-          asm volatile("s_waitcnt lgkmcnt(%0)" ::"n"(NI + MI) : "memory");
+          const unsigned tbn = (unsigned)(it + 1) * 512u;
+          asm volatile("s_waitcnt lgkmcnt(%0)" ::"n"(RD) : "memory");
           __builtin_amdgcn_sched_barrier(0);
+          gn_in_apply(xf0, gt0);
           if (!dbg_on(p, 4)) mma_half(wf0, xf0);
           __builtin_amdgcn_sched_barrier(0);
           if (newgroup || !more) {
@@ -391,16 +452,17 @@
             __builtin_amdgcn_sched_barrier(0);
             if (more) {
               __builtin_amdgcn_s_barrier();
-              reads0(sbn);
+              reads0(sbn, tbn);
             }
           } else {
-            reads0(sbn);
-            asm volatile("s_waitcnt lgkmcnt(%0)" ::"n"(NI + MI) : "memory");
+            reads0(sbn, tbn);
+            asm volatile("s_waitcnt lgkmcnt(%0)" ::"n"(RD) : "memory");
           }
           __builtin_amdgcn_sched_barrier(0);
+          gn_in_apply(xf1, gt1);
           if (!dbg_on(p, 4)) mma_half(wf1, xf1);
           __builtin_amdgcn_sched_barrier(0);
-          if (more) reads1(sbn);
+          if (more) reads1(sbn, tbn);
           ++ing;
         }
       } else {
@@ -686,9 +748,9 @@
 }
 
 template <typename K>
-static int launch_k(K kernel, int smem, DeviceOnce* attr_done, const KP& kp, int tiles, hipStream_t stream, int threads = 256) {
+static int launch_k(K kernel, int smem, DeviceOnce* attr_done, const KP& kp, int tiles, hipStream_t stream, int threads = 256, int smem_cap = 0) {
   if (attr_done->need()) {
-    SDEO_HIP(hipFuncSetAttribute(reinterpret_cast<const void*>(kernel), hipFuncAttributeMaxDynamicSharedMemorySize, smem));
+    SDEO_HIP(hipFuncSetAttribute(reinterpret_cast<const void*>(kernel), hipFuncAttributeMaxDynamicSharedMemorySize, smem_cap > smem ? smem_cap : smem));
     attr_done->mark();
   }
   hipLaunchKernelGGL(kernel, dim3(tiles, 1, kp.splitk), dim3(threads), smem, stream, kp);
@@ -696,12 +758,21 @@
   return 0;
 }
 
-template <int BM, int BN, int ST, bool UPS, bool WS, bool W8 = false, int KPB = 1, bool MX = false, int EPI = EPI_STAGED>
+static constexpr int kLdsBytes = 160 * 1024;
+static constexpr int dma_smem(int bm, int bn, int st, bool w8) { return st * (w8 ? bm * 128 + (bn + 63) / 64 * 4096 : (bm + bn) * 128) + bm * 8; }
+template <int BM, int BN, int ST, bool UPS, bool WS, bool W8 = false, int KPB = 1, bool MX = false, int EPI = EPI_STAGED, bool GNIN = false>
 static int launch_dma(const KP& kp, int tiles, hipStream_t stream) {
   static DeviceOnce done;
-  constexpr int smem = ST * (W8 ? BM * 128 + (BN + 63) / 64 * 4096 : (BM + BN) * 128) + BM * 8;
-  static_assert(smem <= 160 * 1024, "LDS");
-  return launch_k(&conv_gemm_dma_kernel<BM, BN, ST, UPS, WS, W8, KPB, MX, false, EPI>, smem, &done, kp, tiles, stream, WS ? 512 : 256);
+  constexpr int smem = dma_smem(BM, BN, ST, W8);
+  static_assert(smem <= kLdsBytes, "LDS");
+  auto kernel = &conv_gemm_dma_kernel<BM, BN, ST, UPS, WS, W8, KPB, MX, false, EPI, GNIN>;
+  if constexpr (GNIN) {
+    constexpr int cap = smem + kGnInMaxC * 8 < kLdsBytes ? smem + kGnInMaxC * 8 : kLdsBytes;
+    if (!kp.gn_in || smem + kp.Cin * 8 > cap) return fail("conv_gemm: GroupNorm-of-the-input launch without its operands, or a table that does not fit in LDS");
+    return launch_k(kernel, smem + kp.Cin * 8, &done, kp, tiles, stream, 512, cap);
+  } else {
+    return launch_k(kernel, smem, &done, kp, tiles, stream, WS ? 512 : 256);
+  }
 }
 
 typedef int (*MultiLaunch)(const MPArgs& a, int tiles, hipStream_t stream);
@@ -730,7 +801,11 @@
 static constexpr TileCfg dma_tile(const char* name) {
   constexpr bool WS = !(CAPS & CAP_LIGHT);
   TileCfg c{BM, BN, 64, ST, TK_DMA, CAPS | (KPB > 1 ? CAP_GROUPED : 0), KPB, 0, 0, name,
-            &launch_dma<BM, BN, ST, false, WS, false, KPB>, &launch_dma<BM, BN, ST, true, WS, false, KPB>, nullptr, nullptr, {}};
+            &launch_dma<BM, BN, ST, false, WS, false, KPB>, &launch_dma<BM, BN, ST, true, WS, false, KPB>, nullptr, nullptr, {}, {}};
+  if constexpr ((CAPS & CAP_GN_IN) != 0) {
+    static_assert(WS && (KINDS & K_D) != 0, "the GroupNorm-of-the-input form rides on the row's register-direct kind");
+    c.gn_in[EPI_DIRECT] = &launch_dma<BM, BN, ST, false, WS, false, KPB, false, EPI_DIRECT, true>;
+  }
   c.epi[EPI_STAGED] = c.plain;
   if constexpr ((KINDS & K_D) != 0) c.epi[EPI_DIRECT] = &launch_dma<BM, BN, ST, false, WS, false, KPB, false, EPI_DIRECT>;
   if constexpr ((KINDS & K_SK) != 0) c.epi[EPI_SPLITK] = &launch_dma<BM, BN, ST, false, WS, false, KPB, false, EPI_SPLITK>;
@@ -743,16 +818,16 @@
 }
 template <int BM, int BN>
 static constexpr TileCfg generic_tile(const char* name) {
-  return {BM, BN, 32, 2, TK_GENERIC, 0, 1, 0, 0, name, &launch_generic<BM, BN>, &launch_generic<BM, BN>, nullptr, nullptr, {&launch_generic<BM, BN>}};
+  return {BM, BN, 32, 2, TK_GENERIC, 0, 1, 0, 0, name, &launch_generic<BM, BN>, &launch_generic<BM, BN>, nullptr, nullptr, {&launch_generic<BM, BN>}, {}};
 }
 static const TileCfg kTiles[] = {
     dma_tile<128, 128, 3, CAP_MX>("conv_gemm_dma_kernel<128,128,3>"),
     dma_tile<128, 64, 3, CAP_W8 | CAP_MX>("conv_gemm_dma_kernel<128,64,3>"),
-    dma_tile<64, 64, 4, CAP_W8, 1, K_D | K_SK | K_GG>("conv_gemm_dma_kernel<64,64,4>"),
+    dma_tile<64, 64, 4, CAP_W8 | CAP_GN_IN, 1, K_D | K_SK | K_GG>("conv_gemm_dma_kernel<64,64,4>"),
     generic_tile<128, 64>("conv_gemm_kernel<128,64,32,true>"),
     generic_tile<64, 64>("conv_gemm_kernel<64,64,32,true>"),
     dma_tile<256, 128, 3>("conv_gemm_dma_kernel<256,128,3>"),
-    dma_tile<64, 160, 3, CAP_W8 | CAP_MX, 1, K_D | K_SK | K_GN>("conv_gemm_dma_kernel<64,160,3>"),
+    dma_tile<64, 160, 3, CAP_W8 | CAP_MX | CAP_GN_IN, 1, K_D | K_SK | K_GN>("conv_gemm_dma_kernel<64,160,3>"),
     dma_tile<128, 160, 3>("conv_gemm_dma_kernel<128,160,3>"),
     dma_tile<256, 160, 3>("conv_gemm_dma_kernel<256,160,3>"),
     dma_tile<32, 160, 4, CAP_W8>("conv_gemm_dma_kernel<32,160,4>"),
@@ -780,7 +855,7 @@
     dma_tile<128, 64, 6, 0, 2>("conv_gemm_dma_kernel<128,64,6,k2>"),
     dma_tile<64, 64, 6, 0, 2>("conv_gemm_dma_kernel<64,64,6,k2>"),
     dma_tile<128, 128, 4, 0, 2>("conv_gemm_dma_kernel<128,128,4,k2>"),
-    dma_tile<32, 160, 5, 0, 2>("conv_gemm_dma_kernel<32,160,5,k2>"),
+    dma_tile<32, 160, 5, CAP_GN_IN, 2>("conv_gemm_dma_kernel<32,160,5,k2>"),
 };
 static const int kTileCount = (int)std::size(kTiles);
 static bool by_plan_only(const TileCfg& c) { return (c.caps & (CAP_HALO | CAP_LIGHT | CAP_GROUPED)) != 0; }
@@ -920,7 +995,8 @@
   *splitk = pl.splitk;
 }
 
-static int g_last_tile = -1, g_last_splitk = 0, g_last_epilogue = -1;
+static int g_last_tile = -1, g_last_splitk = 0, g_last_epilogue = -1, g_last_gn_in = 0;
+int conv_gemm_last_gn_in() { return g_last_gn_in; }
 void conv_gemm_last_plan(int* tile, int* splitk) { *tile = g_last_tile; *splitk = g_last_splitk; }
 int conv_gemm_last_epilogue() { return g_last_epilogue < 0 ? -1 : g_last_epilogue == EPI_DIRECT ? EPI_DIRECT : EPI_STAGED; }
 int conv_gemm_last_epilogue_mode() { return g_last_epilogue >= EPI_SPLITK ? g_last_epilogue : 0; }
@@ -1063,7 +1139,27 @@
   }
   if (kTiles[pl.tile].kind == TK_HALO) SDEO_CHECK(halo_ok(p, kTiles[pl.tile]), "conv_gemm: halo plan on an ineligible problem");
   pl.epi = epi_kind(p, kp, pl);
+  if (p.gn_in) {
+    SDEO_CHECK(p.gn_in_gamma && p.gn_in_beta && p.gn_in_slots >= 1 && p.gn_in_groups >= 1 && p.Cin % p.gn_in_groups == 0,
+               "conv_gemm: incomplete GroupNorm-of-the-input arguments");
+    kp.gn_in = p.gn_in; kp.gn_in_gamma = p.gn_in_gamma; kp.gn_in_beta = p.gn_in_beta;
+    kp.gn_in_slots = p.gn_in_slots; kp.gn_in_groups = p.gn_in_groups; kp.gn_in_cpg = p.Cin / p.gn_in_groups;
+    kp.gn_in_hw = p.Ho * p.Wo; kp.gn_in_tpg = 256 / p.gn_in_groups; kp.gn_in_eps = p.gn_in_eps;
+  }
   return 0;
+}
+
+static const char* gn_in_refusal(const Plan& pl, int ups, bool w8, const KP& kp) {
+  const TileCfg& c = kTiles[pl.tile];
+  if (w8 || kp.mx_sx) return "fp8-weight and block-scaled operands have no such form";
+  if (kp.K != kp.Cin || kp.stride != 1 || kp.pad != 0 || ups) return "a 1x1 problem at stride 1 only (a larger filter reads the zero padding un-normalised)";
+  if (pl.splitk > 1) return "not under split-K";
+  if (c.kind != TK_DMA || !c.gn_in[pl.epi]) return "the tile has no such instantiation for the launch's epilogue kind";
+  if (kp.gn_in_hw % c.bm) return "the M tile does not divide the pixels of an image";
+  const int g = kp.gn_in_groups;
+  if (g < 4 || g > 64 || (g & (g - 1)) || kp.Cin > kGnInMaxC || kp.gn_in_slots > 128) return "group layout outside what the table build covers (4..64 groups, a power of two; at most 2048 channels, 128 slots)";
+  if (dma_smem(c.bm, c.bn, c.stages, false) + kp.Cin * 8 > kLdsBytes) return "the table does not fit in LDS";
+  return nullptr;
 }
 
 static int dispatch(const Plan& pl, int ups, bool w8, const KP& kp, hipStream_t stream) {
@@ -1073,7 +1169,10 @@
   if (pl.epi != EPI_STAGED && (kp.mx_sx || w8 || ups || !c.epi[pl.epi]))
     return fail("conv_gemm: tile %d has no %s instantiation for this launch", pl.tile, pl.epi == EPI_DIRECT ? "register-direct" : "specialised staged");
   if (pl.epi >= EPI_SPLITK && pl.epi != staged_mode(kp)) return fail("conv_gemm: epilogue kind %d does not match the problem's mode (%d)", pl.epi, staged_mode(kp));
-  const TileLaunch launch = pl.epi != EPI_STAGED ? c.epi[pl.epi] : kp.mx_sx ? c.mx : w8 ? c.w8 : ups ? c.ups : c.plain;
+  if (kp.gn_in) {
+    if (const char* why = gn_in_refusal(pl, ups, w8, kp)) return fail("conv_gemm: GroupNorm of the input on tile %d: %s", pl.tile, why);
+  }
+  const TileLaunch launch = kp.gn_in ? c.gn_in[pl.epi] : pl.epi != EPI_STAGED ? c.epi[pl.epi] : kp.mx_sx ? c.mx : w8 ? c.w8 : ups ? c.ups : c.plain;
   if (!launch) return fail("conv_gemm: tile %d has no %s instantiation", pl.tile, kp.mx_sx ? "block-scaled fp8" : w8 ? "fp8-weight" : "folded-upsample");
   ++g_census[{pl.tile, pl.splitk, kp.mx_sx ? 3 : w8 ? 2 : ups ? 1 : 0, pl.epi, census_flags(kp)}];
   if (int rc = launch(kp, pl.tiles_m * pl.tiles_n, stream)) return rc;
@@ -1092,8 +1191,17 @@
   Plan pl;
   KP kp{};
   if (int rc = prepare(p, pl, kp)) return rc;
-  g_last_tile = pl.tile; g_last_splitk = pl.splitk; g_last_epilogue = pl.epi;
+  g_last_tile = pl.tile; g_last_splitk = pl.splitk; g_last_epilogue = pl.epi; g_last_gn_in = kp.gn_in != nullptr;
   return dispatch(pl, p.ups, p.wscale != nullptr, kp, stream);
+}
+
+bool conv_gemm_plan_has_gn_in(const ConvGemm& p0) {
+  if (!p0.gn_in) return false;
+  const ConvGemm p = mx_view(p0);
+  Plan pl;
+  KP kp{};
+  if (prepare(p, pl, kp)) return false;
+  return gn_in_refusal(pl, p.ups, p.wscale != nullptr, kp) == nullptr;
 }
 
 struct MultiTile { int tile, bm, bn, stages; bool light; MultiLaunch launch; const char* name; };
diff --git a/stablediffusioneo_amd/csrc/conv_inl.h b/stablediffusioneo_amd/csrc/conv_inl.h
--- a/stablediffusioneo_amd/csrc/conv_inl.h
+++ b/stablediffusioneo_amd/csrc/conv_inl.h
@@ -39,7 +39,14 @@
   const unsigned char* mx_sx;
   const unsigned char* mx_sw;
   int mx_ldsx, mx_ldsw;
+  const float* gn_in;
+  const float* gn_in_gamma;
+  const float* gn_in_beta;
+  int gn_in_slots, gn_in_groups, gn_in_cpg, gn_in_hw;
+  int gn_in_tpg;
+  float gn_in_eps;
 };
+constexpr int kGnInMaxC = 2048;
 
 struct MPTable {
   int prefix[kMultiMax];
@@ -696,6 +703,11 @@
 }
 
 template <int OFF>
+__device__ __forceinline__ void lds_read128(f32x4& dst, unsigned addr) {
+  asm volatile("ds_read_b128 %0, %1 offset:%2" : "=v"(dst) : "v"(addr), "n"(OFF) : "memory");
+}
+
+template <int OFF>
 __device__ __forceinline__ void lds_read_w(f16x8& dst, unsigned addr) { lds_read128<OFF>(dst, addr); }
 template <int OFF>
 __device__ __forceinline__ void lds_read_w(uint2& dst, unsigned addr) {
@@ -709,7 +721,7 @@
 
 
 enum TileKind { TK_DMA, TK_GENERIC, TK_HALO };
-enum TileCap { CAP_LIGHT = 1, CAP_GROUPED = 2, CAP_W8 = 4, CAP_MX = 8, CAP_HALO = 16 };
+enum TileCap { CAP_LIGHT = 1, CAP_GROUPED = 2, CAP_W8 = 4, CAP_MX = 8, CAP_HALO = 16, CAP_GN_IN = 32 };
 typedef int (*TileLaunch)(const KP& kp, int tiles, hipStream_t stream);
 struct TileCfg {
   int bm, bn, bk, stages;
@@ -719,6 +731,7 @@
   const char* name;
   TileLaunch plain, ups, w8, mx;
   TileLaunch epi[EPI_KINDS];
+  TileLaunch gn_in[EPI_KINDS];
 };
 constexpr int K_D = 1 << EPI_DIRECT, K_SK = 1 << EPI_SPLITK, K_GG = 1 << EPI_GEGLU, K_GN = 1 << EPI_GN, K_GNB = 1 << EPI_GN_B2;
 const TileCfg& halo_row(int variant);
diff --git a/stablediffusioneo_amd/csrc/gn_affine.h b/stablediffusioneo_amd/csrc/gn_affine.h
--- /dev/null
+++ b/stablediffusioneo_amd/csrc/gn_affine.h
@@ -0,0 +1,38 @@
+#pragma once
+#include "common.h"
+
+namespace sdeo {
+
+__device__ __forceinline__ float2 gn_slot_sum(const float2* __restrict__ src, int nsc, int groups, int l, int tpg) {
+  float ts = 0.f, tq = 0.f;
+  for (int c0 = l; c0 < nsc; c0 += 8 * tpg) {
+    float2 v[8];
+#pragma unroll
+    for (int u = 0; u < 8; ++u) {
+      const int c = c0 + u * tpg;
+      v[u] = c < nsc ? src[(size_t)c * groups] : make_float2(0.f, 0.f);
+    }
+#pragma unroll
+    for (int u = 0; u < 8; ++u) { ts += v[u].x; tq += v[u].y; }
+  }
+  return make_float2(ts, tq);
+}
+
+__device__ __forceinline__ void gn_group_stats(float ts, float tq, int cpg, int HW, float eps, float& mean, float& rstd) {
+#pragma clang fp contract(off)
+  const float inv = 1.0f / ((float)cpg * (float)HW);
+  mean = ts * inv;
+  float var = __builtin_fmaf(-mean, mean, tq * inv);
+  var = var < 0.f ? 0.f : var;
+  rstd = rsqrtf(var + eps);
+}
+
+__device__ __forceinline__ void gn_channel_affine(float mean, float rstd, float gamma, float beta, float& a, float& b) {
+#pragma clang fp contract(off)
+  a = rstd * gamma;
+  b = __builtin_fmaf(-a, mean, beta);
+}
+
+__device__ __forceinline__ float gn_affine_f32(f16 x, float a, float b) { return __builtin_fmaf((float)x, a, b); }
+
+}
diff --git a/stablediffusioneo_amd/csrc/kernels.h b/stablediffusioneo_amd/csrc/kernels.h
--- a/stablediffusioneo_amd/csrc/kernels.h
+++ b/stablediffusioneo_amd/csrc/kernels.h
@@ -41,6 +41,11 @@
   int mx_ldsx = 0, mx_ldsw = 0;
   int res_rows = 0;
   int plan_B = 0;
+  const float* gn_in = nullptr;
+  const float* gn_in_gamma = nullptr;
+  const float* gn_in_beta = nullptr;
+  int gn_in_slots = 0, gn_in_groups = 0;
+  float gn_in_eps = 1e-5f;
 };
 int conv_gemm(const ConvGemm& p, hipStream_t stream);
 inline int conv_pad_after(const ConvGemm& p) { return p.pad_after < 0 ? p.pad : p.pad_after; }
@@ -56,6 +61,8 @@
 int conv_gemm_multi_launch(const ConvGemmMultiPlan& pl, const void* table_dev, const float* scales, hipStream_t stream);
 int conv_gemm_gn_slots(const ConvGemm& p, int cpg);
 bool conv_gemm_plan_is_halo(const ConvGemm& p);
+bool conv_gemm_plan_has_gn_in(const ConvGemm& p);
+int conv_gemm_last_gn_in();
 int conv_gemm_stats_strips(const ConvGemm& p);
 int conv_gemm_read_stamps(unsigned long long* out, int n);
 int conv_halo_read_stamps(unsigned long long* out, int n);
diff --git a/stablediffusioneo_amd/csrc/net.hip b/stablediffusioneo_amd/csrc/net.hip
--- a/stablediffusioneo_amd/csrc/net.hip
+++ b/stablediffusioneo_amd/csrc/net.hip
@@ -35,6 +35,7 @@
   }
   e->cache.configured_anew();
   e->fp8.mx_launches = 0;
+  e->gn_in_launches = 0;
   e->device_bytes = e->ws.slab_bytes + e->fp8.q8_bytes + e->fp8.mx_bytes + e->ws.lora_backup_bytes;
 }
 
@@ -222,6 +223,7 @@
   SDEO_CHECK(latent_h >= maxds && latent_w >= maxds && latent_h % maxds == 0 && latent_w % maxds == 0,
              "sdeo_configure: latent %dx%d must be a positive multiple of %d", latent_h, latent_w, maxds);
   SDEO_CHECK(h->fp8.weight_bits != 8 || h->fp8.q8slab, "sdeo_configure: fp8 weights are packed by sdeo_finalize_weights: call it first");
+  { const char* v = getenv("SDEO_GN_IN"); h->gn_in = !v || atoi(v) != 0; }
   const int rc = configure_impl(h, n, latent_h, latent_w);
   if (rc) free_configured(h);
   return rc;
diff --git a/stablediffusioneo_amd/csrc/net_build.hip b/stablediffusioneo_amd/csrc/net_build.hip
--- a/stablediffusioneo_amd/csrc/net_build.hip
+++ b/stablediffusioneo_amd/csrc/net_build.hip
@@ -23,6 +23,7 @@
   bool gn_next = false;
   const f16* w_ovr = nullptr; const float* b_ovr = nullptr;
   int pad_before = -1, pad_after = -1;
+  const char* gn_in_norm = nullptr; float gn_in_eps = 1e-5f;
 };
 
 struct Builder {
@@ -138,15 +139,29 @@
     p.ln_stats = o.ln->p; p.ln_s = o.ln_s; p.ln_strips = o.ln->strips; p.ln_ld = o.ln->ld; p.ln_c = o.ln->c; p.ln_eps = 1e-5f;
   }
 
-  T conv(const T& x, const std::string& name, int cout, int k, int stride, int ups, const CO& o = CO()) {
+  bool gn_in_fits(const T& x, const std::string& norm, float eps, const std::string& name, int cout, CO o) {
+    if (!e->gn_in || e->autotune || x.gn_slots < 1 || e->fp8.act_bits == 8) return false;
+    const int B = half ? x.n / 2 : x.n;
+    GnArgs ga{nullptr, x.p, nullptr, nullptr, nullptr, x.c, x.ld, B, x.h * x.w, x.c, 32, eps, 0};
+    if (groupnorm_is_single_launch(ga)) return false;
+    if (!W(name + ".weight") || !W(norm + ".weight")) return false;
+    alignas(256) static float standin[64];
+    T y = x.view(); y.c = y.ld = cout;
+    o.gn_in_norm = norm.c_str(); o.gn_in_eps = eps;
+    ConvGemm p = conv_problem(x, y, name, cout, cout, 1, 1, 0, o);
+    if (!p.x) p.x = p.y = reinterpret_cast<f16*>(standin);
+    p.gn_in = standin;
+    if (o.stats) { p.stats_out = standin; p.stats_ld = o.stats->ld; }
+    e->fp8.use_fp8_weights(p, p.plan_B ? p.M / p.B * p.plan_B : p.M, e->ws.slab);
+    return conv_gemm_plan_has_gn_in(p);
+  }
+
+  ConvGemm conv_problem(const T& x, const T& y, const std::string& name, int cout, int cs, int k, int stride, int ups, const CO& o) {
     const WEntry* w = o.w_ovr ? nullptr : W(name + ".weight");
     ConvGemm p;
     const int pad = o.pad_before >= 0 ? o.pad_before : k / 2;
     const int pad_after = o.pad_after >= 0 ? o.pad_after : k / 2;
-    const int hv = ups ? 2 * x.h : x.h, wv = ups ? 2 * x.w : x.w;
-    const int ho = (hv + pad + pad_after - k) / stride + 1, wo = (wv + pad + pad_after - k) / stride + 1;
-    const int cs = o.cout_store > 0 ? o.cout_store : cout;
-    T y = o.out ? o.out->view() : alloc(x.n, ho, wo, cs);
+    const int ho = y.h, wo = y.w;
     const int n = half ? x.n / 2 : x.n;
     if (w && w->ipad != x.c && err.empty()) err = "conv " + name + ": input has " + std::to_string(x.c) + " channels, weight expects " + std::to_string(w->ipad);
     p.x = x.p; p.y = y.p;
@@ -159,6 +174,22 @@
     if (half) p.plan_B = x.n;
     if (o.res_half) p.res_rows = p.M / 2;
     p.ldx = x.ld; p.ldw = p.K; p.ldy = y.ld; p.act = o.act;
+    if (o.gn_in_norm) {
+      p.gn_in = x.gnp; p.gn_in_slots = x.gn_slots; p.gn_in_groups = 32; p.gn_in_eps = o.gn_in_eps;
+      p.gn_in_gamma = vptr(std::string(o.gn_in_norm) + ".weight"); p.gn_in_beta = vptr(std::string(o.gn_in_norm) + ".bias");
+    }
+    return p;
+  }
+
+  T conv(const T& x, const std::string& name, int cout, int k, int stride, int ups, const CO& o = CO()) {
+    const int pad = o.pad_before >= 0 ? o.pad_before : k / 2;
+    const int pad_after = o.pad_after >= 0 ? o.pad_after : k / 2;
+    const int hv = ups ? 2 * x.h : x.h, wv = ups ? 2 * x.w : x.w;
+    const int ho = (hv + pad + pad_after - k) / stride + 1, wo = (wv + pad + pad_after - k) / stride + 1;
+    const int cs = o.cout_store > 0 ? o.cout_store : cout;
+    T y = o.out ? o.out->view() : alloc(x.n, ho, wo, cs);
+    ConvGemm p = conv_problem(x, y, name, cout, cs, k, stride, ups, o);
+    if (p.gn_in && !dry && !share) ++e->gn_in_launches;
     const bool want_gn = o.gn_next && !o.out && !o.scale_host && cs == y.c;
     if (want_gn) reserve_gn_partials(p, y);
     launch_conv(p, o.scale_host, o.stats, want_gn ? &y : nullptr, &o);
@@ -317,11 +348,17 @@
   const int C = blk.cin, H = blk.heads, d = C / H, N = x.n, Tq = x.h * x.w;
   const int TkS = round8(c.context_len);
   b.half = b.share;
-  T g = b.gn(x, p + ".norm", 1e-6f, 0);
-  RowStats st0 = b.alloc_stats(x.rows(), C), st1 = b.alloc_stats(x.rows(), C), st2 = b.alloc_stats(x.rows(), C);
+  const std::string norm = p + ".norm";
+  RowStats st0, st1, st2;
   Builder::CO pi; pi.stats = &st0;
-  T tok = b.conv(g, p + ".proj_in", C, 1, 1, 0, pi);
-  b.release(g);
+  st0.ld = std::max(1, (C + 31) / 32);
+  const bool fused_norm = b.gn_in_fits(x, norm, 1e-6f, p + ".proj_in", C, pi);
+  T g;
+  if (!fused_norm) g = b.gn(x, norm, 1e-6f, 0);
+  st0 = b.alloc_stats(x.rows(), C); st1 = b.alloc_stats(x.rows(), C); st2 = b.alloc_stats(x.rows(), C);
+  if (fused_norm) { pi.gn_in_norm = norm.c_str(); pi.gn_in_eps = 1e-6f; }
+  T tok = b.conv(fused_norm ? x : g, p + ".proj_in", C, 1, 1, 0, pi);
+  if (!fused_norm) b.release(g);
   Builder::CO l1; l1.ln = &st0; l1.ln_s = b.named_v(t + ".attn1.qkv_ln.s");
   T qkv = b.gemm(tok, b.named_w(t + ".attn1.qkv_ln.w"), C, 3 * C, b.named_v(t + ".attn1.qkv_ln.b"), l1);
   T o1 = b.alloc(x.n, x.h, x.w, C);
diff --git a/stablediffusioneo_amd/csrc/net_handle.h b/stablediffusioneo_amd/csrc/net_handle.h
--- a/stablediffusioneo_amd/csrc/net_handle.h
+++ b/stablediffusioneo_amd/csrc/net_handle.h
@@ -113,6 +113,8 @@
   Program prog[P_COUNT];
   std::vector<size_t> ctrl_elems;
   size_t device_bytes = 0;
+  bool gn_in = true;
+  int gn_in_launches = 0;
   bool autotune = false;
   Profiler prof;
 };
diff --git a/stablediffusioneo_amd/csrc/net_weights.hip b/stablediffusioneo_amd/csrc/net_weights.hip
--- a/stablediffusioneo_amd/csrc/net_weights.hip
+++ b/stablediffusioneo_amd/csrc/net_weights.hip
@@ -326,6 +326,7 @@
   return 0;
 }
 int sdeo_debug_mx_launches(sdeo_handle h) { return h ? h->fp8.mx_launches : -1; }
+int sdeo_debug_gn_in_launches(sdeo_handle h) { return h ? h->gn_in_launches : -1; }
 
 int sdeo_set_weight_precision(sdeo_handle h, int bits) {
   SDEO_CHECK(h, "sdeo_set_weight_precision: null handle");
diff --git a/stablediffusioneo_amd/csrc/norm.hip b/stablediffusioneo_amd/csrc/norm.hip
--- a/stablediffusioneo_amd/csrc/norm.hip
+++ b/stablediffusioneo_amd/csrc/norm.hip
@@ -1,5 +1,6 @@
 #include <stdlib.h>
 
+#include "gn_affine.h"
 #include "kernels.h"
 
 namespace sdeo {
@@ -152,17 +153,8 @@
     const int gl = tid / tpg, l = tid - gl * tpg;
     float ts = 0.f, tq = 0.f;
     if (gl < gpb) {
-      const float2* src = reinterpret_cast<const float2*>(partials) + ((size_t)b * nsc * groups + part * gpb + gl);
-      for (int c0 = l; c0 < nsc; c0 += 8 * tpg) {
-        float2 v[8];
-#pragma unroll
-        for (int u = 0; u < 8; ++u) {
-          const int c = c0 + u * tpg;
-          v[u] = c < nsc ? src[(size_t)c * groups] : make_float2(0.f, 0.f);
-        }
-#pragma unroll
-        for (int u = 0; u < 8; ++u) { ts += v[u].x; tq += v[u].y; }
-      }
+      const float2 t2 = gn_slot_sum(reinterpret_cast<const float2*>(partials) + ((size_t)b * nsc * groups + part * gpb + gl), nsc, groups, l, tpg);
+      ts = t2.x; tq = t2.y;
     }
     s_a[tid] = ts;
     s_b[tid] = tq;
@@ -172,12 +164,10 @@
     const int tpg = 256 / gpb;
     float ts = 0.f, tq = 0.f;
     for (int l = 0; l < tpg; ++l) { ts += s_a[tid * tpg + l]; tq += s_b[tid * tpg + l]; }
-    const float inv = 1.0f / ((float)cpg * (float)HW);
-    const float mean = ts * inv;
-    float var = tq * inv - mean * mean;
-    var = var < 0.f ? 0.f : var;
+    float mean, rstd;
+    gn_group_stats(ts, tq, cpg, HW, eps, mean, rstd);
     s_mean[tid] = mean;
-    s_rstd[tid] = rsqrtf(var + eps);
+    s_rstd[tid] = rstd;
   }
   __syncthreads();
 #pragma unroll
@@ -185,9 +175,10 @@
     const int c = tid + k * 256;
     if (c < nvb * 8) {
       const int g = c / cpg;
-      const float a = s_rstd[g] * gpre[k];
+      float a, bb;
+      gn_channel_affine(s_mean[g], s_rstd[g], gpre[k], bpre[k], a, bb);
       s_a[c] = a;
-      s_b[c] = bpre[k] - s_mean[g] * a;
+      s_b[c] = bb;
     }
   }
   __syncthreads();
@@ -202,7 +193,7 @@
       f16x8 o;
 #pragma unroll
       for (int j = 0; j < 8; ++j) {
-        float f = (float)xv[u][j] * a[j] + bb[j];
+        float f = gn_affine_f32(xv[u][j], a[j], bb[j]);
         if (with_silu) f = silu_f(f);
         o[j] = (f16)f;
       }
@@ -214,7 +205,7 @@
     f16x8 o;
 #pragma unroll
     for (int j = 0; j < 8; ++j) {
-      float f = (float)v[j] * a[j] + bb[j];
+      float f = gn_affine_f32(v[j], a[j], bb[j]);
       if (with_silu) f = silu_f(f);
       o[j] = (f16)f;
     }
diff --git a/stablediffusioneo_amd/csrc/sdeo_internal.h b/stablediffusioneo_amd/csrc/sdeo_internal.h
--- a/stablediffusioneo_amd/csrc/sdeo_internal.h
+++ b/stablediffusioneo_amd/csrc/sdeo_internal.h
@@ -55,6 +55,13 @@
                                 const float* beta, int groups, float eps, int with_silu, float* partials, size_t partial_floats, int* slots,
                                 void* stream);
 
+int sdeo_debug_gn_in_conv2d_f16(void* y, int ldy, const void* x, int ldx, const float* partials, int slots, const float* gamma,
+                                const float* beta, int groups, float eps, const void* w_krsc, const float* bias, int n, int h, int w,
+                                int cin, int cout, int ksize, float* stats, int stats_ld, int* strips_out, int fused, void* xnorm,
+                                void* gn_workspace, const void* xs, const void* ws, void* workspace, size_t workspace_bytes,
+                                int* ran_fused, void* stream);
+int sdeo_debug_conv2d_plan_has_gn_in(int n, int h, int w, int cin, int cout, int ksize, int groups, int slots);
+
 int sdeo_debug_gemm_res_rows_f16(void* y, int ldy, const void* x, int ldx, const void* w, int ldw, const float* bias, const void* res,
                                  int ldres, int res_rows, int m, int n, int k, float* stats, int stats_ld, int* strips_out, void* workspace,
                                  size_t workspace_bytes, void* stream);
@@ -79,6 +86,7 @@
 void sdeo_debug_next_weights_fp8(const void* q, const float* scale);
 
 int sdeo_debug_mx_launches(sdeo_handle h);
+int sdeo_debug_gn_in_launches(sdeo_handle h);
 
 const char* sdeo_debug_fake_scribble_profile(const uint8_t* edges, int h, int w, uint8_t* scribble, float* control_chw, void* workspace,
                                              size_t workspace_bytes, void* stream);
diff --git a/stablediffusioneo_amd/ops.py b/stablediffusioneo_amd/ops.py
--- a/stablediffusioneo_amd/ops.py
+++ b/stablediffusioneo_amd/ops.py
@@ -205,6 +205,36 @@
     if want_partials:
         return y, yn, slots.value, part[: n * slots.value * groups * 2].view(n, slots.value, groups, 2)
     return y, yn, slots.value
+
+
+def conv2d_plan_has_gn_in(n, h, w, cin, cout, k=1, groups=32, slots=1):
+    return bool(_lib.load().sdeo_debug_conv2d_plan_has_gn_in(n, h, w, cin, cout, k, groups, slots))
+
+
+def gn_in_conv2d(x, partials, gamma, beta, w_krsc, bias=None, groups=32, eps=1e-5, fused=True, want_stats=False, out=None, w8=None, mx=None):
+    lib = _lib.load()
+    _need_cuda(x, partials, gamma, beta, w_krsc)
+    n, h, w, cin = x.shape
+    cout, k, _, cin_w = w_krsc.shape
+    assert cin == cin_w and w_krsc.is_contiguous() and partials.is_contiguous() and partials.dtype == torch.float32
+    assert partials.shape[0] == n and partials.shape[2] == groups and partials.shape[3] == 2
+    slots = partials.shape[1]
+    y = torch.empty((n, h, w, cout), dtype=torch.float16, device=x.device) if out is None else out
+    assert tuple(y.shape) == (n, h, w, cout)
+    stats_ld = (cout + 31) // 32
+    stats = torch.zeros((n * h * w, stats_ld, 2), dtype=torch.float32, device=x.device) if want_stats else None
+    strips = C.c_int(0)
+    ran = C.c_int(0)
+    xnorm = None if fused else torch.empty((n, h, w, cin), dtype=torch.float16, device=x.device)
+    gws = None if fused else torch.empty(n * groups * 2 + 16, dtype=torch.float32, device=x.device)
+    ws = _ws(max(lib.sdeo_conv2d_workspace_bytes(n, h, w, cin, cout, k, 1, 0), 0 if w8 is None else 64 << 20), x.device)
+    xq, xs, wq, wsc = mx if mx is not None else (None, None, None, None)
+    _arm_fp8(lib, w8)
+    check(lib.sdeo_debug_gn_in_conv2d_f16(ptr(y), _nhwc_ld(y, "out"), ptr(x if mx is None else xq), _nhwc_ld(x, "x"), ptr(partials), slots,
+                                          ptr(gamma), ptr(beta), groups, eps, ptr(w_krsc if mx is None else wq), ptr(bias), n, h, w, cin, cout, k,
+                                          ptr(stats), stats_ld, C.byref(strips), int(fused), ptr(xnorm), ptr(gws), ptr(xs), ptr(wsc),
+                                          ptr(ws), ws.numel(), C.byref(ran), cur_stream()), "gn_in_conv2d")
+    return y, stats, strips.value, bool(ran.value)
 
 
 def conv2d_ex(x, w_krsc, bias=None, res=None, res_rows=0, want_stats=False, ln=None, w8=None):
```
